# sandflow/ffmpeg-ht

Measured on AMD Instinct MI355X. Metric: Mpixels/s HTJ2K decode (4K lossless 5/3) at 1/2/4/8 GPU; IDWT HBM GB/s vs peak, higher is better.
Workload: dtype int32 (int16 storage); 1 GPU; configs[1]: 3840x2160 RGB 8-bit lossless 5/3 + RCT, 64x64 codeblocks, 5 levels, single tile, HT cleanup pass only; 128 frames per step per GPU as 2 concurrent jobs (HIP streams; the frame pipeline keeps that many in flight), device-resident input (codeblock bytes + descriptors) and output (rgb24); jobs=2, distinct_frames=4, block_errors=0

## Files before the change

ffmpeg-ht_amd/csrc/ht_kernels.hpp:

```cpp
#pragma once
#include <hip/hip_runtime.h>
#include <stdint.h>
#include "j2k_plan.h"

namespace htj2k {

struct HtLds {
    uint32_t off_ms, ms_words;
    uint32_t off_vlc, vlc_words;
    uint32_t off_suf, suf_bytes;
    uint32_t off_qinfo, max_qw;
    uint32_t off_E;
    uint32_t off_bm, bm_words;
    uint32_t total;
};

#define HT_ERR_INVALID 1
#define HT_REF_STRIDE 64
#define HT_MEL_SYMS  1344
#define HT_MEL_WORDS (HT_MEL_SYMS / 32 + 2)
#define HT_UVLC_ENTRIES (5 * 64)
#define HT_VSTAGE_PITCH 17
#define HT_VSTAGE_BYTES (64 * HT_VSTAGE_PITCH * 4)

typedef uint16_t ht_sym_t;
__host__ __device__ inline uint32_t ht_nsw(uint32_t Scup) { return (Scup * 8 + 31) / 32 + 2; }
__host__ __device__ inline uint32_t ht_nsp(uint32_t Lref) { return (Lref * 8 + 31) / 32 + 3; }

__host__ __device__ inline uint32_t ht_sym_pack_fields(uint32_t rho, uint32_t ek, uint32_t e1)
{
    uint32_t pk = 0;
    for (int n = 0; n < 4; n++) pk |= (((rho >> n) & 1) + ((ek >> n) & 1) + ((e1 >> n) & 1)) << (2 * n);
    return pk;
}
__device__ __forceinline__ uint32_t ht_sym_unpack(uint32_t s)
{
    const uint32_t pk = s & 0xFF, lo = pk & 0x55, hi = (pk >> 1) & 0x55;
    uint32_t t = (lo | hi) | (hi << 8) | ((lo & hi) << 16);
    t = (t | (t >> 1)) & 0x333333u;
    t = (t | (t >> 2)) & 0x0F0F0Fu;
    return (t & 0xF) | ((t >> 4) & 0xF0) | ((t >> 8) & 0xF00) | ((s >> 8) << 16);
}
__host__ __device__ inline uint32_t ht_qsym_pitch(uint32_t w) { return (((w + 1) >> 1) + 1) & ~1u; }
__host__ __device__ inline uint32_t ht_qsym_words(uint32_t w, uint32_t h) { return (ht_qsym_pitch(w) * ((h + 1) >> 1) + 15) & ~15u; }

__device__ __forceinline__ uint32_t wave_incl_scan_u32(uint32_t v, int lane)
{
    (void)lane;
    int x = (int)v;
    x += __builtin_amdgcn_update_dpp(0, x, 0x111, 0xf, 0xf, false);
    x += __builtin_amdgcn_update_dpp(0, x, 0x112, 0xf, 0xf, false);
    x += __builtin_amdgcn_update_dpp(0, x, 0x114, 0xf, 0xf, false);
    x += __builtin_amdgcn_update_dpp(0, x, 0x118, 0xf, 0xf, false);
    x += __builtin_amdgcn_update_dpp(0, x, 0x142, 0xa, 0xf, false);
    x += __builtin_amdgcn_update_dpp(0, x, 0x143, 0xc, 0xf, false);
    return (uint32_t)x;
}
__device__ __forceinline__ uint32_t wave_last(uint32_t v) { return (uint32_t)__builtin_amdgcn_readlane((int)v, 63); }

__device__ __forceinline__ void wave_lds_fence()
{
    __builtin_amdgcn_fence(__ATOMIC_ACQ_REL, "wavefront");
    __builtin_amdgcn_wave_barrier();
}

__device__ __forceinline__ void ht_ms_clear(uint32_t *p, uint32_t nwords, int lane)
{
    for (uint32_t i = 4u * lane; i < nwords; i += 256) *(uint4 *)(p + i) = make_uint4(0u, 0u, 0u, 0u);
}
__device__ __forceinline__ void ht_ms_ones_tail(uint32_t *p, uint32_t total, uint32_t last_word, int lane)
{
    for (uint32_t i = (total >> 5) + lane; i <= last_word; i += 64) {
        if (i * 32 >= total) p[i] = 0xFFFFFFFFu;
        else p[i] |= 0xFFFFFFFFu << (total & 31);
    }
}

__device__ __forceinline__ uint32_t ht_dequant(uint32_t smag, int transform, int M_b, int roi_shift,
                                               float fscale, int i_step)
{
    uint32_t mag = smag & 0x7FFFFFFFu;
    bool neg = (smag >> 31) != 0;
    if (roi_shift) {
        const uint32_t mask = 0xFFFFFFFFu >> (M_b + 1);
        if ((mag & ~mask) == 0) {
            const uint32_t v = mag << roi_shift;
            neg = neg || (v >> 31) != 0;
            mag = v & 0x7FFFFFFFu;
        }
    }
    if (transform == J2K_DWT53) {
        int v = (int)(mag >> (31 - M_b));
        if (neg) v = -v;
        if (i_step != 32768) {
            long long t = (long long)v * i_step;
            v = (int)(t < 0 ? -((-t) >> 16) : (t >> 16));
        }
        return (uint32_t)v;
    } else if (transform == J2K_DWT97) {
        int v = neg ? -(int)mag : (int)mag;
        return __float_as_uint((float)v * fscale);
    } else {
        int v = neg ? -(int)mag : (int)mag;
        v = (v + 32) >> 6;
        long long t = (long long)v * i_step;
        return (uint32_t)(int)((t + (1 << 15)) >> 16);
    }
}

struct HtSerial {
    uint64_t vbuf; int vbits; uint32_t vword;
    const uint32_t *vlc; uint32_t vlc_words;
    const uint8_t *suf; uint32_t mel_pos, mel_len; uint32_t mel_tmp; int mel_bits;
    int mel_k, mel_run, mel_one;

    __device__ __forceinline__ void vfill()
    {
        if (vbits <= 32) {
            uint32_t wv = vword < vlc_words ? vlc[vword] : 0u;
            vword++;
            vbuf |= (uint64_t)wv << vbits;
            vbits += 32;
        }
    }
    __device__ __forceinline__ uint32_t vpeek(int n) { vfill(); return (uint32_t)vbuf & ((1u << n) - 1); }
    __device__ __forceinline__ void vdrop(int n) { vbuf >>= n; vbits -= n; }
    __device__ __forceinline__ uint32_t vget(int n) { uint32_t v = vpeek(n); vdrop(n); return v; }

    __device__ __forceinline__ int mel_bit()
    {
        if (mel_bits == 0) {
            const bool cond = mel_pos < mel_len;
            mel_bits = (mel_tmp == 0xFF) ? 7 : 8;
            mel_tmp = cond ? suf[mel_pos] : 0xFFu;
            mel_pos += cond;
        }
        mel_bits--;
        return (mel_tmp >> mel_bits) & 1;
    }
    __device__ __forceinline__ int mel_sym()
    {
        static const uint8_t MEL_E[13] = { 0, 0, 0, 1, 1, 1, 2, 2, 2, 3, 3, 4, 5 };
        if (mel_run == 0 && mel_one == 0) {
            int eval = (0x5433222111000ull >> (4 * mel_k)) & 0xF;
            (void)MEL_E;
            if (mel_bit()) {
                mel_run = 1 << eval;
                mel_k = mel_k < 12 ? mel_k + 1 : 12;
            } else {
                mel_run = 0;
                while (eval > 0) { mel_run = 2 * mel_run + mel_bit(); eval--; }
                mel_run &= 0xFF;
                mel_k = mel_k > 0 ? mel_k - 1 : 0;
                mel_one = 1;
            }
        }
        if (mel_run > 0) { mel_run--; return 0; }
        mel_one = 0;
        return 1;
    }
    __device__ __forceinline__ int upfx()
    {
        uint32_t b = vpeek(3);
        int val  = (0x12131215u >> (4 * b)) & 0xF;
        int drop = (0x12131213u >> (4 * b)) & 0xF;
        vdrop(drop);
        return val;
    }
    __device__ __forceinline__ int usfx(int pfx)
    {
        if (pfx < 3) return 0;
        if (pfx == 3) return (int)vget(1);
        return (int)vget(5);
    }
    __device__ __forceinline__ int uext(int sfx) { return sfx >= 28 ? (int)vget(4) : 0; }
};

__device__ __forceinline__ void ht_zero_window(uint32_t *dst, int w, int h, int stride, int lane)
{
    for (int y = 0; y < h; y++)
// ... 1232 lines not shown
                }
                dst[(size_t)y * stride + x] = ht_dequant(v, transform, M_b, roi_shift, fscale, i_step);
            }
    }
}


__device__ __forceinline__ void ht_unstuff_backward_step8(uint2 dq, uint32_t k0, uint32_t n, uint32_t first_or,
                                                          uint32_t *out, int lane, uint32_t &base, uint32_t &carry)
{
    const uint32_t k = k0 + 8 * lane;
    uint32_t lo = __builtin_bswap32(dq.y), hi = __builtin_bswap32(dq.x);
    if (k == 0) lo |= first_or;
    int nv = 8;
    if (k0 + 512 > n) {
        nv = min(max((int)n - (int)k, 0), 8);
        const int nl = min(nv, 4), nh = nv - nl;
        lo = nl == 4 ? lo : (nl ? lo & (0xFFFFFFFFu >> (32 - 8 * nl)) : 0u);
        hi = nh == 4 ? hi : (nh ? hi & (0xFFFFFFFFu >> (32 - 8 * nh)) : 0u);
    }
    const uint32_t ll = lo & 0x7F7F7F7Fu, lh = hi & 0x7F7F7F7Fu;
    const uint32_t Al = (ll + 0x70707070u) & lo & 0x80808080u, Ah = (lh + 0x70707070u) & hi & 0x80808080u;
    const uint32_t Bl = (ll + 0x01010101u) & 0x80808080u, Bh = (lh + 0x01010101u) & 0x80808080u;
    uint32_t prevA = ht_dpp_left(Ah >> 24);
    if (lane == 0) prevA = carry;
    carry = (uint32_t)__builtin_amdgcn_readlane((int)(Ah >> 24), 63);
    uint32_t fl = Bl & ((Al << 8) | prevA), fh = Bh & __builtin_amdgcn_alignbyte(Ah, Al, 3);
    if (nv < 8) {
        const int nl = min(nv, 4), nh = nv - nl;
        fl = nl == 4 ? fl : (nl ? fl & (0xFFFFFFFFu >> (32 - 8 * nl)) : 0u);
        fh = nh == 4 ? fh : (nh ? fh & (0xFFFFFFFFu >> (32 - 8 * nh)) : 0u);
    }
    ht_squeeze_place<false>(lo, hi, fl, fh, nv, out, lane, base);
}

__device__ __forceinline__ uint32_t ht_unstuff_backward(const uint8_t *__restrict__ top, uint32_t n, uint32_t first_or,
                                                        uint32_t *out, int lane)
{
    uint32_t base = 0, carry = 0x80;
    for (uint32_t k0 = 0; k0 < n; k0 += 512) {
        const uint32_t k = k0 + 8 * lane;
        uint2 dq = make_uint2(0u, 0u);
        if (k < n) __builtin_memcpy(&dq, top - k - 7, 8);
        ht_unstuff_backward_step8(dq, k0, n, first_or, out, lane, base, carry);
    }
    return base;
}

__device__ __forceinline__ uint32_t ht_unstuff_forward7(const uint8_t *__restrict__ src, uint32_t n, uint32_t *out, int lane)
{
    uint32_t base = 0, carry = 0;
    for (uint32_t p0 = 0; p0 * 8 < n; p0 += 64) {
        const uint32_t i = (p0 + lane) * 8;
        uint2 dq = make_uint2(0u, 0u);
        if (i < n) __builtin_memcpy(&dq, src + i, 8);
        ht_unstuff_fwd_step8<false>(dq, p0, n, out, lane, base, carry);
    }
    return base;
}


template <int LPB>
__device__ __forceinline__ uint32_t grp_incl_scan_u32(uint32_t v)
{
    int x = (int)v;
    x += __builtin_amdgcn_update_dpp(0, x, 0x111, 0xf, 0xf, false);
    x += __builtin_amdgcn_update_dpp(0, x, 0x112, 0xf, 0xf, false);
    x += __builtin_amdgcn_update_dpp(0, x, 0x114, 0xf, 0xf, false);
    x += __builtin_amdgcn_update_dpp(0, x, 0x118, 0xf, 0xf, false);
    if (LPB >= 32) x += __builtin_amdgcn_update_dpp(0, x, 0x142, 0xa, 0xf, false);
    if (LPB >= 64) x += __builtin_amdgcn_update_dpp(0, x, 0x143, 0xc, 0xf, false);
    return (uint32_t)x;
}
template <int LPB>
__device__ __forceinline__ uint32_t grp_last(uint32_t v, int lane)
{
    return (uint32_t)__builtin_amdgcn_ds_bpermute((lane | (LPB - 1)) << 2, (int)v);
}
template <bool OR_SEM, int LPB>
__device__ __forceinline__ void ht_squeeze_place_g(uint32_t lo, uint32_t hi, uint32_t fl, uint32_t fh, int nv,
                                                   uint32_t *out, int lane, uint32_t &base)
{
    const uint32_t tot = 8u * (uint32_t)nv - (uint32_t)__builtin_popcount(fl) - (uint32_t)__builtin_popcount(fh);
    while (__ballot(fh != 0) != 0) {
        if (fh) {
            const uint32_t k = 31u - (uint32_t)__builtin_clz(fh), bit = 1u << k, m = bit - 1u;
            uint32_t nh = (hi & m) | ((hi >> 1) & ~m);
            if (OR_SEM) nh |= hi & bit;
            hi = nh;
            fh &= m;
        }
    }
    while (__ballot(fl != 0) != 0) {
        if (fl) {
            const uint32_t k = 31u - (uint32_t)__builtin_clz(fl), bit = 1u << k, m = bit - 1u;
            uint32_t nl = (lo & m) | (__builtin_amdgcn_alignbit(hi, lo, 1) & ~m);
            if (OR_SEM) nl |= lo & bit;
            lo = nl;
            hi >>= 1;
            fl &= m;
        }
    }
    const uint32_t incl = grp_incl_scan_u32<LPB>(tot);
    const uint32_t off = base + incl - tot;
    if (nv > 0) {
        const uint32_t sh = off & 31;
        const uint64_t t = (uint64_t)lo << sh, u = (uint64_t)hi << sh;
        uint32_t *o = out + (off >> 5);
        atomicOr(o, (uint32_t)t);
        atomicOr(o + 1, (uint32_t)(t >> 32) | (uint32_t)u);
        if (sh + tot + (OR_SEM ? 1u : 0u) > 64) atomicOr(o + 2, (uint32_t)(u >> 32));
    }
    base += grp_last<LPB>(incl, lane);
}
__device__ __forceinline__ uint32_t ht_first_bytes(uint32_t v, int n) { return n >= 4 ? v : (n > 0 ? v & (0xFFFFFFFFu >> (32 - 8 * n)) : 0u); }
template <int LPB>
__device__ __forceinline__ void ht_unstuff_backward_step8_g(uint2 dq, uint32_t k0, uint32_t n, uint32_t first_or,
                                                            uint32_t *out, int lane, uint32_t &base, uint32_t &carry)
{
    const int gl = lane & (LPB - 1);
    const uint32_t k = k0 + 8 * gl;
    const int nv = min(max((int)n - (int)k, 0), 8);
    uint32_t lo = __builtin_bswap32(dq.y), hi = __builtin_bswap32(dq.x);
    if (k == 0) lo |= first_or;
    lo = ht_first_bytes(lo, nv); hi = ht_first_bytes(hi, nv - 4);
    const uint32_t ll = lo & 0x7F7F7F7Fu, lh = hi & 0x7F7F7F7Fu;
    const uint32_t Al = (ll + 0x70707070u) & lo & 0x80808080u, Ah = (lh + 0x70707070u) & hi & 0x80808080u;
    const uint32_t Bl = (ll + 0x01010101u) & 0x80808080u, Bh = (lh + 0x01010101u) & 0x80808080u;
    uint32_t prevA = ht_dpp_left(Ah >> 24);
    if (gl == 0) prevA = carry;
    carry = grp_last<LPB>(Ah >> 24, lane);
    const uint32_t fl = ht_first_bytes(Bl & ((Al << 8) | prevA), nv), fh = ht_first_bytes(Bh & __builtin_amdgcn_alignbyte(Ah, Al, 3), nv - 4);
    ht_squeeze_place_g<false, LPB>(lo, hi, fl, fh, nv, out, lane, base);
}
template <int LPB>
__device__ __forceinline__ void ht_unstuff_fwd7_step8_g(uint2 dq, uint32_t p0, uint32_t n, uint32_t *out, int lane,
                                                        uint32_t &base, uint32_t &carry)
{
    const int gl = lane & (LPB - 1);
    const int nv = min(max((int)n - (int)(p0 + 8 * gl), 0), 8);
    const uint32_t lo = ht_first_bytes(dq.x, nv), hi = ht_first_bytes(dq.y, nv - 4);
    uint32_t prev = ht_dpp_left(hi >> 24);
    if (gl == 0) prev = carry;
    carry = grp_last<LPB>(hi >> 24, lane);
    const uint32_t Pl = (lo << 8) | prev, Ph = __builtin_amdgcn_alignbyte(hi, lo, 3);
    const uint32_t fl = ht_first_bytes(((Pl & 0x7F7F7F7Fu) + 0x01010101u) & Pl & 0x80808080u, nv);
    const uint32_t fh = ht_first_bytes(((Ph & 0x7F7F7F7Fu) + 0x01010101u) & Ph & 0x80808080u, nv - 4);
    ht_squeeze_place_g<false, LPB>(lo, hi, fl, fh, nv, out, lane, base);
}

template <int LPB>
__global__ void __launch_bounds__(64)
k_ht_unstuff_g(const J2kBlock *__restrict__ blocks, int nblocks, const uint8_t *__restrict__ bytes,
               uint32_t *__restrict__ vlc_u, uint32_t *__restrict__ mel_u, uint32_t lds_words)
{
    extern __shared__ __align__(16) uint32_t sw[];
    constexpr int G = 64 / LPB;
    const int lane = threadIdx.x, gl = lane & (LPB - 1);
    const int bi = (int)blockIdx.x * G + lane / LPB;
    J2kBlock b;
    memset(&b, 0, sizeof(b));
    if (bi < nblocks) b = blocks[bi];
    const uint8_t *D = bytes + b.data_off;
    const uint32_t Lcup = b.lcup;
    bool ok = bi < nblocks && b.npasses != 0 && Lcup >= 2;
    uint2 pv[2];
#pragma unroll
    for (int j = 0; j < 2; j++) {
        const long long o = (long long)b.data_off + Lcup - 9 - (8 * LPB * j + 8 * gl);
        pv[j] = make_uint2(0u, 0u);
        if (ok && o >= 0) __builtin_memcpy(&pv[j], bytes + o, 8);
    }
    uint32_t Scup = 0;
    if (ok) Scup = ((uint32_t)D[Lcup - 1] << 4) + (D[Lcup - 2] & 0x0F);
    ok = ok && !(Scup < 2 || Scup > Lcup || Scup > 4079);
    const uint32_t nsw = ht_nsw(Scup);
    ok = ok && 2 * nsw <= lds_words;
    uint32_t *vlO = vlc_u + (b.data_off >> 2), *meO = mel_u + (b.data_off >> 2);
    uint32_t *sv = sw + (size_t)(lane / LPB) * lds_words;

    if (ok) for (uint32_t i = gl; i < nsw; i += LPB) sv[i] = 0;
    __syncthreads();
    {
        const uint8_t *top = D + Lcup - 2;
        const uint32_t n = ok ? Scup - 1 : 0u;
        uint32_t base = 0, carry = 0x80;
#pragma unroll
        for (int j = 0; j < 2; j++)
            if (__ballot((uint32_t)(8 * LPB * j) < n) != 0) ht_unstuff_backward_step8_g<LPB>(pv[j], 8 * LPB * j, n, 0x0F, sv, lane, base, carry);
        for (uint32_t k0 = 16 * LPB; __ballot(k0 < n) != 0; k0 += 8 * LPB) {
            const uint32_t k = k0 + 8 * gl;
            uint2 dq = make_uint2(0u, 0u);
            if (k < n) __builtin_memcpy(&dq, top - k - 7, 8);
            ht_unstuff_backward_step8_g<LPB>(dq, k0, n, 0x0F, sv, lane, base, carry);
        }
    }
    __syncthreads();
    if (ok) for (uint32_t i = gl; i < nsw; i += LPB) vlO[i] = sv[i];

    const int rem = b.npasses % 3, plhd = rem ? b.npasses - rem : b.npasses - 3;
    const uint32_t Lref = b.lref, nsp = ht_nsp(Lref);
    const bool ref = ok && b.npasses - plhd > 1 && Lref > 0 && 2 * nsp <= lds_words;
    if (__ballot(ref) == 0) return;
    uint32_t *ss = sv, *sr = sv + nsp;
    __syncthreads();
    if (ref) for (uint32_t i = gl; i < 2 * nsp; i += LPB) sv[i] = 0;
    __syncthreads();
    {
        const uint32_t n = ref ? Lref : 0u;
        uint32_t base = 0, carry = 0;
        for (uint32_t p0 = 0; __ballot(p0 < n) != 0; p0 += 8 * LPB) {
            const uint32_t i = p0 + 8 * gl;
            uint2 dq = make_uint2(0u, 0u);
            if (i < n) __builtin_memcpy(&dq, D + Lcup + i, 8);
            ht_unstuff_fwd7_step8_g<LPB>(dq, p0, n, ss, lane, base, carry);
        }
        base = 0; carry = 0x80;
        const uint8_t *top = D + Lcup + Lref - 1;
        for (uint32_t k0 = 0; __ballot(k0 < n) != 0; k0 += 8 * LPB) {
            const uint32_t k = k0 + 8 * gl;
            uint2 dq = make_uint2(0u, 0u);
            if (k < n) __builtin_memcpy(&dq, top - k - 7, 8);
            ht_unstuff_backward_step8_g<LPB>(dq, k0, n, 0, sr, lane, base, carry);
        }
    }
    __syncthreads();
    if (ref) for (uint32_t i = gl; i < nsp; i += LPB) {
        vlO[nsw + i] = ss[i];
        meO[nsw + i] = sr[i];
    }
}

__global__ void __launch_bounds__(64)
k_ht_unstuff(const J2kBlock *__restrict__ blocks, int nblocks, const uint8_t *__restrict__ bytes,
             uint32_t *__restrict__ vlc_u, uint32_t *__restrict__ mel_u, uint32_t lds_words)
{
    extern __shared__ __align__(16) uint32_t sw[];
    const int lane = threadIdx.x;
    if ((int)blockIdx.x >= nblocks) return;
    const J2kBlock b = blocks[blockIdx.x];
    if (b.npasses == 0 || b.lcup < 2) return;
    const uint8_t *D = bytes + b.data_off;
    const uint32_t Lcup = b.lcup;
    uint2 pv[2];
#pragma unroll
    for (int j = 0; j < 2; j++) {
        const long long o = (long long)b.data_off + Lcup - 9 - (512 * j + 8 * lane);
        pv[j] = make_uint2(0u, 0u);
        if (o >= 0) __builtin_memcpy(&pv[j], bytes + o, 8);
    }
    const uint32_t Scup = (uint32_t)__builtin_amdgcn_readfirstlane((int)(((uint32_t)D[Lcup - 1] << 4) + (D[Lcup - 2] & 0x0F)));
    if (Scup < 2 || Scup > Lcup || Scup > 4079) return;
    const uint32_t nsw = ht_nsw(Scup);
    if (2 * nsw > lds_words) return;
    uint32_t *vlO = vlc_u + (b.data_off >> 2), *meO = mel_u + (b.data_off >> 2);
    uint32_t *sv = sw;

    for (uint32_t i = lane; i < nsw; i += 64) sw[i] = 0;
    __syncthreads();

    {
        const uint8_t *top = D + Lcup - 2;
        const uint32_t n = Scup - 1;
        uint32_t base = 0, carry = 0x80;
#pragma unroll
        for (int j = 0; j < 2; j++)
            if (512u * j < n) ht_unstuff_backward_step8(pv[j], 512 * j, n, 0x0F, sv, lane, base, carry);
        for (uint32_t k0 = 1024; k0 < n; k0 += 512) {
            const uint32_t k = k0 + 8 * lane;
            uint2 dq = make_uint2(0u, 0u);
            if (k < n) __builtin_memcpy(&dq, top - k - 7, 8);
            ht_unstuff_backward_step8(dq, k0, n, 0x0F, sv, lane, base, carry);
        }
    }

    __syncthreads();
    for (uint32_t i = lane; i < nsw; i += 64) vlO[i] = sv[i];

    const int rem = b.npasses % 3, plhd = rem ? b.npasses - rem : b.npasses - 3;
    if (b.npasses - plhd > 1 && b.lref > 0) {
        const uint32_t Lref = b.lref, nsp = ht_nsp(Lref);
        if (2 * nsp > lds_words) return;
        uint32_t *ss = sw, *sr = sw + nsp;
        __syncthreads();
        for (uint32_t i = lane; i < 2 * nsp; i += 64) sw[i] = 0;
        __syncthreads();
        ht_unstuff_forward7(D + Lcup, Lref, ss, lane);
        ht_unstuff_backward(D + Lcup + Lref - 1, Lref, 0, sr, lane);
        __syncthreads();
        for (uint32_t i = lane; i < nsp; i += 64) {
            vlO[nsw + i] = ss[i];
            meO[nsw + i] = sr[i];
        }
    }
}

template <typename MT, bool MAGREF>
__global__ void __launch_bounds__(64, (sizeof(MT) == 4 && !MAGREF) ? 6 : 4)
k_ht_refine(const J2kBlock *__restrict__ blocks, const uint32_t *__restrict__ ref_list, int nref,
            const uint8_t *__restrict__ bytes, const ht_sym_t *__restrict__ qsym, const uint32_t *__restrict__ qoff,
            const uint32_t *__restrict__ vlc_u, const uint32_t *__restrict__ mel_u,
            uint64_t *__restrict__ refbits, const uint32_t *__restrict__ roff)
{
    constexpr int MB = (int)sizeof(MT) * 8;
    const int li = blockIdx.x * 64 + threadIdx.x;
    if (li >= nref) return;
    const uint32_t bi = ref_list[li];
    const J2kBlock b = blocks[bi];
    const int w = b.w, h = b.h, qw = (w + 1) >> 1, qh = (h + 1) >> 1;
    uint64_t *out = refbits + roff[bi];
    for (int y = 0; y < 3 * h; y++) out[(size_t)y * HT_REF_STRIDE] = 0;
    if (b.npasses == 0 || b.lcup < 2 || w > MB) return;
    const uint8_t *D = bytes + b.data_off;
    const uint32_t Scup = ((uint32_t)D[b.lcup - 1] << 4) + (D[b.lcup - 2] & 0x0F);
    if (Scup < 2 || Scup > b.lcup || Scup > 4079) return;
    const int rem = b.npasses % 3, plhd = rem ? b.npasses - rem : b.npasses - 3;
    const int z_blk = b.npasses - plhd;
    if (z_blk <= 1) return;
    const bool causal = (b.flags & J2K_CBLK_VSC) != 0;
    const ht_sym_t *qs = qsym + qoff[bi];
    const uint32_t nsw = ht_nsw(Scup), nsp = b.lref ? ht_nsp(b.lref) : 0;
    const uint32_t *spw = vlc_u + (b.data_off >> 2) + nsw, *mrw = mel_u + (b.data_off >> 2) + nsw;
    const MT wmask = w >= MB ? (MT)~(MT)0 : (MT)(((MT)1 << w) - 1);

    struct Bits {
        const uint32_t *p; uint32_t n, idx; uint64_t buf; int cnt; uint32_t q0, q1, q2, q3, left; uint4 nx;
        __device__ __forceinline__ uint4 fetch(uint32_t i) const
        {
            uint4 v = make_uint4(0u, 0u, 0u, 0u);
            if (i < n) {
                __builtin_memcpy(&v, p + i, 16);
                if (i + 1 >= n) v.y = 0;
                if (i + 2 >= n) v.z = 0;
                if (i + 3 >= n) v.w = 0;
            }
            return v;
        }
        __device__ __forceinline__ void init(const uint32_t *q, uint32_t nw)
        {
            p = q; n = nw; buf = 0; cnt = 0;
            const uint4 v = fetch(0);
            q0 = v.x; q1 = v.y; q2 = v.z; q3 = v.w; left = 4;
            nx = fetch(4); idx = 8;
        }
        __device__ __forceinline__ void top_up()
        {
            buf |= (uint64_t)q0 << cnt;
            cnt += 32;
            q0 = q1; q1 = q2; q2 = q3;
            if (--left == 0) {
                q0 = nx.x; q1 = nx.y; q2 = nx.z; q3 = nx.w; left = 4;
                nx = fetch(idx); idx += 4;
            }
        }
        __device__ __forceinline__ uint32_t get()
        {
            const uint32_t bit = (uint32_t)buf & 1u;
            buf >>= 1; cnt--;
            return bit;
        }
    } sp, mr;
    sp.init(spw, nsp);
    if (MAGREF) mr.init(mrw, nsp);

    const uint32_t qpitch = ht_qsym_pitch((uint32_t)w);
    auto two_quads = [](uint32_t s2, int q, MT &top, MT &bot) {
        const uint32_t r2 = (s2 | (s2 >> 1)) & 0x00550055u;
        top |= (MT)((r2 & 1u) | ((r2 >> 3) & 2u) | ((r2 >> 14) & 4u) | ((r2 >> 17) & 8u)) << (2 * q);
        bot |= (MT)(((r2 >> 2) & 1u) | ((r2 >> 5) & 2u) | ((r2 >> 16) & 4u) | ((r2 >> 19) & 8u)) << (2 * q);
    };
    auto quad_rows = [&](int qy, MT &top, MT &bot) {
        top = 0; bot = 0;
        if (qy >= qh) return;
        const uint32_t *row = (const uint32_t *)(qs + (size_t)qy * qpitch);
        if ((qpitch & 7) == 0) {
            for (int q = 0; q < qw; q += 8) {
                const uint4 s8 = *(const uint4 *)(row + (q >> 1));
                two_quads(s8.x, q, top, bot);
                two_quads(s8.y, q + 2, top, bot);
                two_quads(s8.z, q + 4, top, bot);
                two_quads(s8.w, q + 6, top, bot);
            }
        } else {
            for (int q = 0; q < qw; q += 2) two_quads(row[q >> 1], q, top, bot);
        }
        top &= wmask; bot &= wmask;
        if (2 * qy + 1 >= h) bot = 0;
    };

    MT a_top, a_bot;
    quad_rows(0, a_top, a_bot);
    MT Mup = 0;
    for (int i0 = 0; i0 < h; i0 += 4) {
        MT b_top, b_bot, c_top, c_bot;
        quad_rows(i0 / 2 + 1, b_top, b_bot);
        quad_rows(i0 / 2 + 2, c_top, c_bot);
        const MT S0 = a_top, S1 = a_bot, S2 = b_top, S3 = b_bot, S4 = c_top;
        MT R0 = 0, R1 = 0, R2 = 0, R3 = 0, G0 = 0, G1 = 0, G2 = 0, G3 = 0, Q0 = 0, Q1 = 0, Q2 = 0, Q3 = 0;
        const int gh = min(4, h - i0);
        {
            auto smear = [](MT x) -> MT { return x | (MT)(x << 1) | (x >> 1); };
            const bool dn0 = !causal || gh != 1, dn1 = !causal || gh != 2, dn2 = !causal || gh != 3, dn3 = !causal || gh != 4;
            MT s0 = S0, s1 = S1, s2 = S2, s3 = S3;
            MT T0 = smear(Mup) | (MT)(S0 << 1) | (S0 >> 1) | (dn0 ? smear(S1) : (MT)0);
            MT T1 = smear(S0) | (MT)(S1 << 1) | (S1 >> 1) | (dn1 ? smear(S2) : (MT)0);
            MT T2 = smear(S1) | (MT)(S2 << 1) | (S2 >> 1) | (dn2 ? smear(S3) : (MT)0);
            MT T3 = smear(S2) | (MT)(S3 << 1) | (S3 >> 1) | (dn3 ? smear(S4) : (MT)0);
            const uint32_t m0 = dn0 ? 7u : 3u, m1 = dn1 ? 7u : 3u, m2 = dn2 ? 7u : 3u, m3 = dn3 ? 7u : 3u;
            uint32_t rprev = 0;
            for (int j0 = 0; j0 < w; j0 += 4) {
                uint32_t rc4[4] = { 0, 0, 0, 0 };
                if (sp.cnt <= 32) sp.top_up();
#pragma unroll
                for (int jj = 0; jj < 4; jj++) {
                    const int j = j0 + jj;
                    if (j < w) {
                        const uint32_t RP = rprev << 1;
                        uint32_t rcur = 0;
                        if (gh > 0 && !((uint32_t)s0 & 1u) && ((((uint32_t)T0 & 1u) | (RP & m0)) != 0) && sp.get()) rcur |= 1u;
                        if (gh > 1 && !((uint32_t)s1 & 1u) && ((((uint32_t)T1 & 1u) | ((RP >> 1) & m1) | (rcur & 1u)) != 0) && sp.get()) rcur |= 2u;
                        if (gh > 2 && !((uint32_t)s2 & 1u) && ((((uint32_t)T2 & 1u) | ((RP >> 2) & m2) | (rcur & 2u)) != 0) && sp.get()) rcur |= 4u;
                        if (gh > 3 && !((uint32_t)s3 & 1u) && ((((uint32_t)T3 & 1u) | ((RP >> 3) & m3) | (rcur & 4u)) != 0) && sp.get()) rcur |= 8u;
                        R0 |= (MT)(rcur & 1u) << j; R1 |= (MT)((rcur >> 1) & 1u) << j;
                        R2 |= (MT)((rcur >> 2) & 1u) << j; R3 |= (MT)(rcur >> 3) << j;
                        rc4[jj] = rcur;
                        rprev = rcur;
                        s0 >>= 1; s1 >>= 1; s2 >>= 1; s3 >>= 1;
                        T0 >>= 1; T1 >>= 1; T2 >>= 1; T3 >>= 1;
                    }
                }
// ... 175 lines not shown
            uint64_t mw;
            uint32_t n7 = 0;
            if (!slow) {
                const uint32_t hi = __builtin_amdgcn_perm(pfB, pfA, 0x01020304u), lo = __builtin_amdgcn_perm(pfC, pfB, 0x01020304u);
                mw = (((uint64_t)hi << 32) | lo) << o;
            } else {
                uint32_t prev = 0, total = 0;
                mw = 0;
#pragma unroll
                for (int j = -1; j < 7; j++) {
                    const int p = mb + j;
                    const uint32_t raw = ((j < 3 ? pfA >> (8 * (j + 1)) : pfB >> (8 * (j - 3)))) & 0xFF;
                    const uint32_t v = p >= mlim - 1 ? 0xFFu : (p == mlim - 2 ? raw | 0x0Fu : raw);
                    if (j >= 0) {
                        const uint32_t n = prev == 0xFF ? 7u : 8u;
                        mw = (mw << n) | (v & ((1u << n) - 1));
                        total += n;
                        n7 |= (8u - n) << j;
                    }
                    prev = p < 0 ? 0u : v;
                }
                mw <<= (64 - total) + (o - (n7 & 1));
            }
            uint32_t used_all = 0;
#pragma unroll
            for (int cw = 0; cw < 6; cw++) {
                const int eval = (int)((0x5433222111000ull >> (4 * mel_k)) & 0xF);
                const int b = (int)(mw >> 63);
                const int run = b ? (1 << eval) : (eval ? (int)((mw << 1) >> (64 - eval)) : 0);
                const int nsy = run + (b ? 0 : 1);
                if (mcnt + nsy <= 64) {
                    if (!b) msyms |= 1ull << ((mcnt + run) & 63);
                    mcnt += nsy;
                    const int used = b ? 1 : 1 + eval;
                    mw <<= used; used_all += used;
                    mel_k = b ? (mel_k < 12 ? mel_k + 1 : 12) : (mel_k > 0 ? mel_k - 1 : 0);
                }
            }
            if (!slow) {
                mrb += used_all;
            } else {
                uint32_t L = 0, before = 0, cum = 8 - o;
#pragma unroll
                for (int j = 0; j < 6; j++) {
                    const bool ge = used_all >= cum;
                    L += ge;
                    before = ge ? cum : before;
                    cum += 8 - ((n7 >> (j + 1)) & 1);
                }
                mrb = L ? (uint32_t)(mb + (int)L) * 8 + ((n7 >> L) & 1) + (used_all - before) : mrb + used_all;
            }
            const uint8_t *pm = mraw + min((int)(mrb >> 3), mlim) - 1;
            __builtin_memcpy(&pfA, pm, 4);
            __builtin_memcpy(&pfB, pm + 4, 4);
            __builtin_memcpy(&pfC, pm + 8, 4);
        }
        uint64_t vwin;
        {
            const uint32_t kw = (vpos >> 5) & 15, sh = vpos & 31;
            const uint32_t a0 = vst[kw], a1 = vst[(kw + 1) & 15], a2 = vst[(kw + 2) & 15];
            vwin = ((uint64_t)__builtin_amdgcn_alignbit(a2, a1, sh) << 32) | __builtin_amdgcn_alignbit(a1, a0, sh);
        }
        uint32_t m = (uint32_t)msyms, mused = 0;
        uint32_t a = (uint32_t)vwin, aused = 0;
        int rho[2], uoff[2];
        uint32_t pk[2];
#pragma unroll
        for (int k = 0; k < 2; k++) {
            const bool en = active && (k == 0 || pair);
            const int q = qx + k;
            const int ra = ra_next;
            const int rar = (row && en && q + 1 < qw) ? (int)myrho[q + 1] : 0;
            const int ctx = row0 ? ctx_run
                                 : ((((ra >> 1) | (ral >> 3)) & 1) | ((((rho_left >> 2) | (rho_left >> 3)) & 1) << 1) |
                                    ((((ra >> 3) | (rar >> 1)) & 1) << 2));
            const bool mq = en && ctx == 0;
            const int msym = (int)(m & 1);
            m >>= mq ? 1 : 0; mused += mq ? 1 : 0;
            const bool dec = en && (ctx != 0 || msym != 0);
            const uint32_t e = dec ? table[(ctx << 7) | (a & 0x7F)] : 0u;
            const uint32_t len = (e >> 1) & 7;
            a >>= len; aused += len;
            uoff[k] = e & 1; rho[k] = (e >> 4) & 0xF; pk[k] = e >> 8;
            if (en) {
                rho_left = rho[k];
                ral = ra;
                ra_next = rar;
                ctx_run = ((rho[k] | (rho[k] >> 1)) & 1) | (((rho[k] >> 2) & 1) << 1) | (((rho[k] >> 3) & 1) << 2);
            }
        }
        uint32_t u32w = (uint32_t)(vwin >> aused), uused;
        const bool both = uoff[0] && uoff[1];
        const bool mq2 = row0 && both;
        const int mel2 = (int)(m & 1);
        mused += mq2 ? 1 : 0;
        const int mode = (mq2 && !mel2) ? 4 : (uoff[0] | (uoff[1] << 1));
        const uint32_t ue = utbl[(mode << 6) | (u32w & 63)];
        const int p1 = ue & 7, p2 = (ue >> 3) & 7;
        uint32_t d = (ue >> 6) & 7;
        u32w >>= d; uused = d;
        d = (ue >> 9) & 7;
        const int s1 = (int)(u32w & ((1u << d) - 1)); u32w >>= d; uused += d;
        d = (ue >> 12) & 7;
        const int s2 = (int)(u32w & ((1u << d) - 1)); u32w >>= d; uused += d;
        d = s1 >= 28 ? 4u : 0u;
        const int x1 = (int)(u32w & ((1u << d) - 1)); u32w >>= d; uused += d;
        d = s2 >= 28 ? 4u : 0u;
        const int x2 = (int)(u32w & ((1u << d) - 1)); uused += d;
        const int bias = (mq2 && mel2) ? 2 : 0;
        const int u1 = uoff[0] ? bias + p1 + s1 + 4 * x1 : 0;
        const int u2 = uoff[1] ? bias + p2 + s2 + 4 * x2 : 0;
        if (active) {
            vpos += aused + uused;
            msyms >>= mused; mcnt -= (int)mused;
            myrho[qx] = (uint8_t)rho[0];
            if (pair) myrho[qx + 1] = (uint8_t)rho[1];
        }
        ost[t & (CAD - 1)] = pk[0] | ((uint32_t)u1 << 8) | (pk[1] << 16) | ((uint32_t)u2 << 24);
        qx += 2;
        if (active && qx >= qw) {
            qx = 0; row++;
            rho_left = 0; ral = 0;
            ra_next = (int)myrho[0];
        }
    }
    if (max_it > 0) flush((max_it - 1) / CAD);
}


#define HT_VLC2_VPITCH 18
#define HT_VLC2_LDS (4096 + 1024 + HT_VLC_NARROW_WAVES * 64 * (HT_VLC2_VPITCH + HT_VLC_OUT_PITCH) * 4)

__host__ __device__ inline uint32_t ht_uvlc_entry2_from(uint32_t p1, uint32_t p2, uint32_t lp, uint32_t d1, uint32_t d2)
{
    return lp | (d1 << 5) | (p1 << 8) | ((lp + d1) << 11) | (d2 << 16) | ((lp + d1 + d2) << 19) | (p2 << 24);
}
__host__ __device__ inline uint32_t ht_uvlc_entry2(int mode, uint32_t v)
{
    const uint32_t e = ht_uvlc_entry(mode, v);
    return ht_uvlc_entry2_from(e & 7, (e >> 3) & 7, (e >> 6) & 7, (e >> 9) & 7, (e >> 12) & 7);
}
__device__ __forceinline__ uint32_t ht_uvlc_entry2_mode4(uint32_t v)
{
    const uint32_t b = v & 7;
    const uint32_t p1 = (0x12131215u >> (4 * b)) & 0xF;
    uint32_t lp = (0x12131213u >> (4 * b)) & 0xF, p2;
    if (p1 > 2) { p2 = ((v >> lp) & 1) + 1; lp += 1; }
    else { const uint32_t b2 = (v >> lp) & 7; p2 = (0x12131215u >> (4 * b2)) & 0xF; lp += (0x12131213u >> (4 * b2)) & 0xF; }
    const uint32_t d1 = p1 < 3 ? 0u : (p1 == 3 ? 1u : 5u);
    const uint32_t d2 = p1 > 2 ? 0u : (p2 < 3 ? 0u : (p2 == 3 ? 1u : 5u));
    return ht_uvlc_entry2_from(p1, p2, lp, d1, d2);
}

__global__ void __launch_bounds__(64 * HT_VLC_NARROW_WAVES)
k_ht_vlc2(const J2kBlock *__restrict__ blocks, int nblocks, const uint8_t *__restrict__ bytes,
          const uint16_t *__restrict__ g_tables, ht_sym_t *__restrict__ qsym,
          const uint32_t *__restrict__ qoff,
          const uint32_t *__restrict__ vlc_u, uint32_t *__restrict__ sink)
{
    extern __shared__ __align__(16) uint8_t smem[];
    uint16_t *tbl = (uint16_t *)smem;
    uint32_t *utbl = (uint32_t *)(smem + 4096);
    constexpr int CAD = 8;
    constexpr int VPITCH = HT_VLC2_VPITCH, OPITCH = HT_VLC_OUT_PITCH;
    const int lane = threadIdx.x & 63, wv = threadIdx.x >> 6;
    uint32_t *vstage = (uint32_t *)(smem + 4096 + 1024) + wv * 64 * (VPITCH + OPITCH);
    uint32_t *ostage = vstage + 64 * VPITCH;
    const int bi = blockIdx.x * blockDim.x + threadIdx.x;
    for (int i = threadIdx.x; i < 2048; i += blockDim.x) {
        const uint32_t e = g_tables[i], rho = (e >> 4) & 0xF;
        const uint32_t ne = (e & 0xF) | (((rho >> 1) & 1) << 4) | (((rho >> 3) & 1) << 5) | ((((rho >> 2) | (rho >> 3)) & 1) << 6) |
                            (ht_sym_pack_fields(rho, (e >> 8) & 0xF, (e >> 12) & 0xF) << 8);
        const int ctx = (i >> 7) & 7, bits = i & 127;
        const int dst = i < 1024 ? i : 1024 + (bits | ((ctx & 1) << 7) | (((ctx >> 2) & 1) << 8) | (((ctx >> 1) & 1) << 9));
        tbl[dst] = (uint16_t)ne;
    }
    for (int i = threadIdx.x; i < 4 * 64; i += blockDim.x)
        utbl[i] = ht_uvlc_entry2(i >> 6, (uint32_t)(i & 63));

    int qw = 0, qh = 0;
    uint32_t doff = 0;
    ht_sym_t *qout = qsym;
    const uint8_t *mraw = bytes + 16;
    int mlim = 0;
    if (bi < nblocks) {
        const J2kBlock b = blocks[bi];
        bool ok = b.npasses != 0 && b.lcup >= 2;
        uint32_t Scup = 0;
        if (ok) {
            const uint8_t *D = bytes + b.data_off;
            Scup = ((uint32_t)D[b.lcup - 1] << 4) + (D[b.lcup - 2] & 0x0F);
            ok = !(Scup < 2 || Scup > b.lcup || Scup > 4079);
        }
        if (ok && ((b.w + 1u) >> 1) <= 32u) {
            qw = (b.w + 1) >> 1;
            qh = (b.h + 1) >> 1;
            qout = qsym + qoff[bi];
            doff = b.data_off >> 2;
            mraw = bytes + b.data_off + (b.lcup - Scup);
            mlim = (int)Scup;
        }
    }
    const int ppr = (qw + 1) >> 1;
    const int n_it = qh * ppr;
    int max_it = n_it;
#pragma unroll
    for (int o = 32; o; o >>= 1) max_it = max(max_it, __shfl_xor(max_it, o));
    const uint32_t my_lo = (uint32_t)(uintptr_t)qout, my_hi = (uint32_t)((uintptr_t)qout >> 32);
    __syncthreads();

    const uint32_t *vsrc = vlc_u + doff;
    uint32_t vpos = 4;
    uint32_t *vst = vstage + lane * VPITCH;
    uint32_t *ost = ostage + lane * OPITCH;
    uint4 nxv = make_uint4(0u, 0u, 0u, 0u), nxw = make_uint4(0u, 0u, 0u, 0u);
    uint32_t hw = 16, pw = 0;
    bool pend = false;
    uint64_t msyms = 0; int mcnt = 0; uint32_t mrb = 0; int mel_k = 0;
    uint32_t pfA, pfB, pfC;
    __builtin_memcpy(&pfA, mraw - 1, 4);
    __builtin_memcpy(&pfB, mraw + 3, 4);
    __builtin_memcpy(&pfC, mraw + 7, 4);
    if (qh > 0) {
#pragma unroll
        for (int jx = 0; jx < 4; jx++) {
            uint4 q;
            __builtin_memcpy(&q, vsrc + 4 * jx, 16);
            vst[4 * jx] = q.x; vst[4 * jx + 1] = q.y; vst[4 * jx + 2] = q.z; vst[4 * jx + 3] = q.w;
            if (jx == 0) { vst[16] = q.x; vst[17] = q.y; }
        }
    }
    auto flush = [&](int win) {
#pragma unroll
        for (int p = 0; p < 2; p++) {
            const int c = 32 * p + (lane >> 1), part = lane & 1;
            const uint32_t *src = ostage + c * OPITCH + 4 * part;
            const uint4 v = make_uint4(src[0], src[1], src[2], src[3]);
            const uint32_t c_lo = (uint32_t)__builtin_amdgcn_ds_bpermute(4 * c, (int)my_lo);
            const uint32_t c_hi = (uint32_t)__builtin_amdgcn_ds_bpermute(4 * c, (int)my_hi);
            const uint32_t c_nit = (uint32_t)__builtin_amdgcn_ds_bpermute(4 * c, n_it);
            uint32_t *dst = (uint32_t *)(((uintptr_t)c_hi << 32) | c_lo) + (size_t)win * CAD + 4 * part;
            typedef uint32_t u32x4 __attribute__((ext_vector_type(4)));
            typedef __attribute__((address_space(1))) u32x4 g_u32x4;
            u32x4 vv; vv.x = v.x; vv.y = v.y; vv.z = v.z; vv.w = v.w;
            *(g_u32x4 *)(uintptr_t)((uint32_t)(win * CAD) < c_nit ? dst : sink + 4 * part) = vv;
        }
    };

    int row = 0, qx = 0;
    uint32_t ctx_run = 0;
    uint32_t lf10 = 0;
    uint32_t Dlo = 0, Dhi = 0, Mlo = 0, Mhi = 0;
    const uint8_t *tb1 = (const uint8_t *)(tbl + 1024);
    auto pass = [&](int t, auto main_tag) {
        constexpr bool MAIN = decltype(main_tag)::value;
        const bool active = MAIN || t < n_it;
        const bool row0 = !MAIN && row == 0;
        const bool pair = MAIN || qx + 1 < qw;
        if ((t & 1) == 0) {
            if (pend) {
                uint32_t *r = vst + (pw & 15);
                r[0] = nxv.x; r[1] = nxv.y; r[2] = nxv.z; r[3] = nxv.w;
                if (!(pw & 15)) { vst[16] = nxv.x; vst[17] = nxv.y; }
                r = vst + ((pw + 4) & 15);
                r[0] = nxw.x; r[1] = nxw.y; r[2] = nxw.z; r[3] = nxw.w;
            }
            pend = (int)(hw - (vpos >> 5)) < 8;
            if (pend) {
                __builtin_memcpy(&nxv, vsrc + hw, 16);
                __builtin_memcpy(&nxw, vsrc + hw + 4, 16);
                pw = hw;
                hw += 8;
            }
            if ((t & (CAD - 1)) == 0 && t) flush(t / CAD - 1);
        }
        if (__ballot(mcnt < 3) != 0 && mcnt <= 32) {
            const int mb = (int)(mrb >> 3);
            const uint32_t o = mrb & 7;
            const uint32_t a0 = mb ? pfA : (pfA & ~0xFFu);
            const uint32_t anyff = ((~a0 - 0x01010101u) & a0 & 0x80808080u) | ((~pfB - 0x01010101u) & pfB & 0x80808080u);
            const bool slow = anyff != 0 || mb + 10 > mlim;
            uint64_t mw;
            uint32_t n7 = 0;
            if (!slow) {
                const uint32_t hi = __builtin_amdgcn_perm(pfB, pfA, 0x01020304u), lo = __builtin_amdgcn_perm(pfC, pfB, 0x01020304u);
                mw = (((uint64_t)hi << 32) | lo) << o;
            } else {
                uint32_t prev = 0, total = 0;
                mw = 0;
#pragma unroll
                for (int j = -1; j < 7; j++) {
                    const int p = mb + j;
                    const uint32_t raw = ((j < 3 ? pfA >> (8 * (j + 1)) : pfB >> (8 * (j - 3)))) & 0xFF;
                    const uint32_t v = p >= mlim - 1 ? 0xFFu : (p == mlim - 2 ? raw | 0x0Fu : raw);
                    if (j >= 0) {
                        const uint32_t n = prev == 0xFF ? 7u : 8u;
                        mw = (mw << n) | (v & ((1u << n) - 1));
                        total += n;
                        n7 |= (8u - n) << j;
                    }
                    prev = p < 0 ? 0u : v;
                }
                mw <<= (64 - total) + (o - (n7 & 1));
            }
            uint32_t used_all = 0;
#pragma unroll
            for (int cw = 0; cw < 6; cw++) {
                const int eval = (int)((0x5433222111000ull >> (4 * mel_k)) & 0xF);
                const int b = (int)(mw >> 63);
                const int run = b ? (1 << eval) : (eval ? (int)((mw << 1) >> (64 - eval)) : 0);
                const int nsy = run + (b ? 0 : 1);
                if (mcnt + nsy <= 64) {
                    if (!b) msyms |= 1ull << ((mcnt + run) & 63);
                    mcnt += nsy;
                    const int used = b ? 1 : 1 + eval;
                    mw <<= used; used_all += used;
                    mel_k = b ? (mel_k < 12 ? mel_k + 1 : 12) : (mel_k > 0 ? mel_k - 1 : 0);
                }
            }
            if (!slow) {
                mrb += used_all;
            } else {
                uint32_t L = 0, before = 0, cum = 8 - o;
#pragma unroll
                for (int j = 0; j < 6; j++) {
                    const bool ge = used_all >= cum;
                    L += ge;
                    before = ge ? cum : before;
                    cum += 8 - ((n7 >> (j + 1)) & 1);
                }
                mrb = L ? (uint32_t)(mb + (int)L) * 8 + ((n7 >> L) & 1) + (used_all - before) : mrb + used_all;
            }
            const uint8_t *pm = mraw + min((int)(mrb >> 3), mlim) - 1;
            __builtin_memcpy(&pfA, pm, 4);
            __builtin_memcpy(&pfB, pm + 4, 4);
            __builtin_memcpy(&pfC, pm + 8, 4);
        }
        uint32_t lo, hi;
        {
            const uint32_t *wp = (const uint32_t *)((const uint8_t *)vst + ((vpos >> 3) & 60u));
            const uint32_t a0 = wp[0], a1 = wp[1], a2 = wp[2];
            lo = __builtin_amdgcn_alignbit(a1, a0, vpos);
            hi = __builtin_amdgcn_alignbit(a2, a1, vpos);
        }
        uint32_t m = (uint32_t)msyms;
        uint32_t e0, e1, mused;
        {
            const bool en0 = active;
            uint32_t ad = row0 ? ((lo & 0x7Fu) << 1) | (ctx_run << 8)
                               : ((lo & 0x7Fu) << 1) | ((Dlo & 3u) << 8) | lf10;
            const uint32_t mq = (en0 && ad < 0x100u) ? 1u : 0u;
            const uint32_t et = *(const uint16_t *)((row0 ? (const uint8_t *)tbl : tb1) + ad);
            e0 = __umul24(et, (m | ~mq) & (MAIN ? 1u : (uint32_t)en0));
            m >>= mq; mused = mq;
            if (row0) {
                const uint32_t f = e0 >> 8, tt = (f | (f >> 1)) & 0x55u;
                if (en0) ctx_run = ((tt | (tt >> 2)) & 1u) | ((tt >> 3) & 2u) | ((tt >> 4) & 4u);
            }
            const bool en1 = active && pair;
            const uint32_t len0 = (e0 >> 1) & 7u;
            const uint32_t bits1 = __builtin_amdgcn_ubfe(lo, len0, 7u) << 1;
            ad = row0 ? bits1 | (ctx_run << 8) : bits1 | ((Dlo & 0xCu) << 6) | ((e0 & 0x40u) << 4);
            const uint32_t mq1 = (en1 && ad < 0x100u) ? 1u : 0u;
            const uint32_t et1 = *(const uint16_t *)((row0 ? (const uint8_t *)tbl : tb1) + ad);
            e1 = __umul24(et1, (m | ~mq1) & (MAIN ? 1u : (uint32_t)en1));
            m >>= mq1; mused += mq1;
            if (row0) {
                const uint32_t f = e1 >> 8, tt = (f | (f >> 1)) & 0x55u;
                if (en1) ctx_run = ((tt | (tt >> 2)) & 1u) | ((tt >> 3) & 2u) | ((tt >> 4) & 4u);
            }
            if (MAIN || en1) lf10 = (e1 & 0x40u) << 4;
            else if (en0) lf10 = (e0 & 0x40u) << 4;
            const uint32_t X = ((e0 >> 4) & 3u) | (((e1 >> 4) & 3u) << 2);
            const uint32_t sh = MAIN ? 4u : 2u * ((uint32_t)en0 + (uint32_t)en1);
            Mlo = __builtin_amdgcn_alignbit(Mhi, Mlo, sh);
            Mhi = __builtin_amdgcn_alignbit(X, Mhi, sh);
            Dlo = __builtin_amdgcn_alignbit(Dhi, Dlo, 4u);
            Dhi >>= 4;
        }
        const uint32_t aused = ((e0 >> 1) & 7u) + ((e1 >> 1) & 7u);
        const uint32_t w = __builtin_amdgcn_alignbit(hi, lo, aused);
        uint32_t ue = utbl[(w & 63u) | ((e0 & 1u) << 6) | ((e1 & 1u) << 7)];
        uint32_t bias = 0;
        if (!MAIN) {
            const bool mq2 = row0 && (e0 & e1 & 1u);
            if (__ballot(mq2) != 0) {
                const uint32_t mel2 = m & 1u;
                if (mq2) {
                    mused += 1;
                    if (mel2) bias = 0x02000200u; else ue = ht_uvlc_entry2_mode4(w & 63u);
                }
            }
        }
        const uint32_t s1 = __builtin_amdgcn_ubfe(w, ue, __builtin_amdgcn_ubfe(ue, 5u, 3u));
        const uint32_t s2 = __builtin_amdgcn_ubfe(w, ue >> 11, __builtin_amdgcn_ubfe(ue, 16u, 3u));
        uint32_t uused = __builtin_amdgcn_ubfe(ue, 19u, 5u);
        uint32_t out = __builtin_amdgcn_perm(e1, e0, 0x0C050C01u) + (ue & 0x07000700u) + (s1 << 8) + (s2 << 24) + bias;
        if (__ballot(s1 >= 28u || s2 >= 28u) != 0) {
            const uint32_t d1x = s1 >= 28u ? 4u : 0u, d2x = s2 >= 28u ? 4u : 0u;
            const uint32_t x1 = __builtin_amdgcn_ubfe(w, uused, d1x), x2 = __builtin_amdgcn_ubfe(w, uused + d1x, d2x);
            out += (x1 << 10) + (x2 << 26);
            uused += d1x + d2x;
        }
        if (active) {
            vpos += aused + uused;
            msyms >>= mused; mcnt -= (int)mused;
        }
        ost[t & (CAD - 1)] = out;
        qx += 2;
        if (active && qx >= qw) {
            const uint64_t I = (((uint64_t)Mhi << 32) | Mlo) >> (64 - 2 * qw);
            const uint64_t Dn = ((I | (I << 1)) & 0x5555555555555555ull) | ((I | (I >> 1)) & 0xAAAAAAAAAAAAAAAAull);
            Dlo = (uint32_t)Dn; Dhi = (uint32_t)(Dn >> 32);
            Mlo = 0; Mhi = 0;
            qx = 0; row++;
            lf10 = 0; ctx_run = 0;
        }
    };
    int t_a = ppr, t_b = n_it, odd = qw & 1;
#pragma unroll
    for (int o = 32; o; o >>= 1) {
        t_a = max(t_a, __shfl_xor(t_a, o));
        t_b = min(t_b, __shfl_xor(t_b, o));
// ... 12 lines not shown
```

ffmpeg-ht_amd/csrc/htj2k_device.hip:

```cpp
#include <hip/hip_runtime.h>
#include <stdarg.h>
#include <stdio.h>
#include <stdlib.h>
#include <string.h>
#include <algorithm>
#include <atomic>
#include <chrono>
#include <mutex>
#include <thread>
#include <vector>

#include "../../include/htj2k_amd.h"
#include "j2k_plan.h"
#include "ht_cxtvlc_rows.h"
#include "ht_kernels.hpp"
#include "dwt_kernels.hpp"
#include "pack_kernels.hpp"
#include "dwt_stream.hpp"
#include "mq_kernels.hpp"

using namespace htj2k;

__global__ void __launch_bounds__(256) k_gather(const J2kSeg *__restrict__ segs, const uint32_t *__restrict__ first_seg, int ngroups,
                                                 const uint8_t *__restrict__ pkt, const uint8_t *__restrict__ lit,
                                                 uint8_t *__restrict__ pool)
{
    const int g = blockIdx.x * 4 + (threadIdx.x >> 6), lane = threadIdx.x & 63;
    if (g >= ngroups) return;
    const uint32_t s1 = first_seg[g + 1];
    for (uint32_t s = first_seg[g]; s < s1; s++) {
        const J2kSeg sg = segs[s];
        const uint8_t *src = ((sg.flags & J2K_SEG_LIT) ? lit : pkt) + sg.src;
        uint8_t *dst = pool + sg.dst;
        const uint32_t head = min(sg.len, (uint32_t)(-(intptr_t)dst & 3));
        if ((uint32_t)lane < head) dst[lane] = src[lane];
        const uint32_t body = (sg.len - head) >> 2, tail0 = head + 4 * body;
        const uint8_t *bs = src + head;
        const uint32_t sh = (uint32_t)((uintptr_t)bs & 3);
        const uint32_t *al = (const uint32_t *)(bs - sh);
        uint32_t *out = (uint32_t *)(dst + head);
        for (uint32_t k = lane; k < body; k += 64) {
            const uint32_t lo = al[k], hi = sh ? al[k + 1] : 0u;
            out[k] = __builtin_amdgcn_alignbyte(hi, lo, sh);
        }
        if ((uint32_t)lane < sg.len - tail0) dst[tail0 + lane] = src[tail0 + lane];
        if ((sg.flags & J2K_SEG_TERM) && lane < 2) dst[sg.len + lane] = 0xFF;
    }
}

#define LOG_ERROR 16
#define LOG_WARNING 24
#define LOG_INFO 32

struct DevBuf {
    void *p = nullptr;
    size_t cap = 0;
    int ensure(size_t n)
    {
        if (n <= cap) return 0;
        if (p) (void)hipFree(p);
        p = nullptr; cap = 0;
        size_t want = n + n / 8 + 256;
        if (hipMalloc(&p, want) != hipSuccess) { p = nullptr; return HTJ2K_ERR_ENOMEM; }
        cap = want;
        static const bool poison = getenv("HTJ2K_POISON") && atoi(getenv("HTJ2K_POISON"));
        if (poison) {
            (void)hipMemset(p, 0xA5, want);
            (void)hipDeviceSynchronize();
        }
        return 0;
    }
    void release() { if (p) (void)hipFree(p); p = nullptr; cap = 0; }
};

struct HostBuf {
    void *p = nullptr;
    size_t cap = 0;
    int device = 0;
    void *ensure(size_t n)
    {
        if (n <= cap) return p;
        if (hipSetDevice(device) != hipSuccess) return nullptr;
        if (p) (void)hipHostFree(p);
        p = nullptr; cap = 0;
        const size_t want = n + n / 4 + 4096;
        if (hipHostMalloc(&p, want, hipHostMallocDefault) != hipSuccess) { p = nullptr; return nullptr; }
        cap = want;
        return p;
    }
    void release() { if (p) (void)hipHostFree(p); p = nullptr; cap = 0; }
};

struct htj2k_ctx {
    htj2k_opts opts;
    int device = 0;
    char devname[256];
    htj2k_log_fn log = nullptr;
    void *log_opaque = nullptr;
    uint16_t *d_tables = nullptr;
    J2kParser *probe_parser = nullptr;
    htj2k_job *own_job = nullptr;
    int idwt_mode = 3;
    int fuse_pack = 1;
    int idwt_x3 = 1;
    int ht_pair = 1;
    int ht_multi = 1;
    int idwt_pk = 1;
    int ll16_test_bits = 16;
    int ll16 = 1;
    int coef16 = 1;
    int ht_mode = 1;
    int max_dyn_lds = 64 * 1024;
    int parse_threads = 0;
    int packet_threads = 1;
    int device_gather = 1;
    std::mutex log_mutex;
    std::atomic<int> refs{1};
};

struct LevelLaunch {
    int type, level;
    int count;
    size_t table_off;
    int max_lh, max_lv, min_l;
    double alg_bytes;
    double hbm_bytes = 0;
    int nc = 0;
    int outk = -1;
    bool all_fast = false;
    int pk_bits = 0;
};

struct FrameSlot {
    J2kParser *parser = nullptr;
    const J2kPlan *plan = nullptr;
    HostBuf h_pkt;
    const uint8_t *h2d_src = nullptr;
    bool h2d_own = false;
    size_t pkt_base = 0;
    HostBuf h_bytes;
    float ms_stage = 0, ms_parse = 0;
    uint32_t block_base = 0, tc_base = 0, sample_base = 0;
    size_t bytes_base = 0;
    DevBuf d_out[4];
    OutPlanes out;
};

struct htj2k_job {
    std::vector<FrameSlot> frames;
    int nframes = 0;
    std::vector<J2kBlock> blocks;
    std::vector<J2kTileComp> tilecomps;
    std::vector<int> tc_frame;
    size_t nbytes = 0, nsamples = 0;
    hipStream_t stream = nullptr;
    hipEvent_t ev[6] = { nullptr, nullptr, nullptr, nullptr, nullptr, nullptr };
    std::vector<hipEvent_t> lev_ev;
    int lev_ev_used = 0;
    std::vector<double> lev_bytes, lev_hbm;
    DevBuf d_bytes, d_blocks, d_status, d_coef, d_t0, d_t1, d_desc, d_qsym, d_qoff, d_vlcu, d_melu, d_reflist, d_roff, d_refbits;
    bool pair_ok = false;
    int multi_nb = 0;
    int multi_t = 0;
    bool coef16_ok = false;
    bool coef_is16 = false;
    int ht_bpw = 0;
    bool ll16_run = false;
    bool ll16_checked = true;
    bool force_ll32 = false;
    int ll16_fallbacks = 0;
    int nht = 0;
    std::vector<MqWave> mqwaves;
    size_t mq_scratch_units = 0;
    uint32_t mq_planes = 1;
    DevBuf d_mqwaves, d_mqscratch;
    bool dev_gather = false;
    DevBuf d_pkt, d_lit, d_gsegs, d_ggroups;
    std::vector<J2kSeg> gsegs;
    std::vector<uint32_t> ggroups;
    std::vector<uint8_t> lit;
    size_t pkt_bytes = 0;
    bool pkt_h2d_issued = false;
    std::vector<uint32_t> qoff;
    std::vector<uint32_t> reflist, roff;
    size_t nrefmasks = 0;
    uint32_t ref_max_w = 0;
    uint32_t ref_max_h = 0;
    uint32_t max_lref = 0;
    size_t nquads = 0;
    HtLds lds_ext;
    uint32_t max_qw = 1;
    std::vector<uint8_t> h_desc;
    std::vector<uint8_t> h_desc_dev;
    std::vector<LevelLaunch> launches_generic, launches_tile;
    std::vector<LevelLaunch> launches_fused;
    std::vector<uint8_t> tile_fusable;
    std::vector<uint8_t> plane_fused;
    bool any_fusable = false;
    int pk_used = 0;
    bool pk_run = false;
    int pk_bits = 0;
    bool x3_ok = false;
    size_t x3_tab[3] = { 0, 0, 0 };
    int x3_count = 0, x3_lh[3] = { 0, 0, 0 }, x3_lv2 = 0;
    double x3_alg = 0, x3_hbm = 0;
    bool fused_last = false;
    size_t pack_off = 0; int npack = 0; int pack_maxw = 0, pack_maxh = 0;
    HtLds lds;
    int uploaded = 0, ran = 0;
    std::vector<int> final_buf;
    std::vector<int> final_eff;
    bool tile_ok = true;
};

static void clog(htj2k_ctx *c, int level, const char *fmt, ...)
{
    char buf[512];
    va_list ap;
    if (!c || !c->log) return;
    va_start(ap, fmt);
    vsnprintf(buf, sizeof buf, fmt, ap);
    va_end(ap);
    c->log(c->log_opaque, level, buf);
}

static void parser_log_tramp(void *opaque, int level, const char *msg)
{
    htj2k_ctx *c = (htj2k_ctx *)opaque;
    if (c && c->log) {
        std::lock_guard<std::mutex> lk(c->log_mutex);
        c->log(c->log_opaque, level, msg);
    }
}

#define HIP_TRY(c, expr)                                                                      \
    do {                                                                                      \
        hipError_t e_ = (expr);                                                               \
        if (e_ != hipSuccess) {                                                               \
            clog(c, LOG_ERROR, "HIP error %s at %s:%d (%s)\n", hipGetErrorString(e_), __FILE__, __LINE__, #expr); \
            return e_ == hipErrorOutOfMemory ? HTJ2K_ERR_ENOMEM : HTJ2K_ERR_EXTERNAL;         \
        }                                                                                     \
    } while (0)

static uint16_t h_tables[2][1024];
static void tbl_row(int t, int ctx, int rho, int uoff, int ek, int e1, int cwd, int len)
{
    uint16_t v = (uint16_t)(uoff | (len << 1) | (rho << 4) | (ek << 8) | (e1 << 12));
    for (int hi = 0; hi < (1 << (7 - len)); hi++)
        h_tables[t][(ctx << 7) | (hi << len) | cwd] = v;
}
#define DROW0(c, r, u, k, o, w, l) tbl_row(0, c, r, u, k, o, w, l);
#define DROW1(c, r, u, k, o, w, l) tbl_row(1, c, r, u, k, o, w, l);
static void build_tables()
{
    HT_CXTVLC_ROWS0(DROW0)
    HT_CXTVLC_ROWS1(DROW1)
}

extern "C" const char *htj2k_version(void) { return "htj2k-amd 0.1 (gfx950)"; }

extern "C" int htj2k_open(const htj2k_opts *opts, htj2k_ctx **out)
{
    int ndev = 0;
    if (!out) return HTJ2K_ERR_EINVAL;
    *out = nullptr;
    if (hipGetDeviceCount(&ndev) != hipSuccess || ndev <= 0)
        return HTJ2K_ERR_ENOSYS;
    htj2k_ctx *c = new (std::nothrow) htj2k_ctx();
    if (!c) return HTJ2K_ERR_ENOMEM;
    memset(&c->opts, 0, sizeof(c->opts));
    c->opts.req_pix_fmt = HTJ2K_PIX_NONE;
    if (opts) c->opts = *opts;
    c->device = c->opts.device_id;
    if (c->device < 0 || c->device >= ndev) { delete c; return HTJ2K_ERR_EINVAL; }
    if (hipSetDevice(c->device) != hipSuccess) { delete c; return HTJ2K_ERR_ENOSYS; }
    hipDeviceProp_t prop;
    if (hipGetDeviceProperties(&prop, c->device) != hipSuccess) { delete c; return HTJ2K_ERR_ENOSYS; }
    snprintf(c->devname, sizeof(c->devname), "%s", prop.gcnArchName);
    c->max_dyn_lds = (int)prop.sharedMemPerBlock;
    build_tables();
    if (hipMalloc((void **)&c->d_tables, sizeof(h_tables)) != hipSuccess ||
        hipMemcpy(c->d_tables, h_tables, sizeof(h_tables), hipMemcpyHostToDevice) != hipSuccess) {
        delete c;
        return HTJ2K_ERR_ENOSYS;
    }
    c->probe_parser = j2k_parser_new();
    if (!c->probe_parser) { (void)hipFree(c->d_tables); delete c; return HTJ2K_ERR_ENOMEM; }
    const char *hm = getenv("HTJ2K_HT");
    if (hm && !strcmp(hm, "fused")) c->ht_mode = 0;
    if (hm && !strcmp(hm, "split")) c->ht_mode = 1;
    const char *m = getenv("HTJ2K_IDWT");
    if (m && !strcmp(m, "generic")) c->idwt_mode = 0;
    if (m && !strcmp(m, "tile")) c->idwt_mode = 1;
    if (m && !strcmp(m, "stream")) c->idwt_mode = 3;
    const char *l16 = getenv("HTJ2K_LL16");
    if (l16) c->ll16 = atoi(l16) ? 1 : 0;
    const char *pk = getenv("HTJ2K_PK");
    if (pk) c->idwt_pk = atoi(pk) ? 1 : 0;
    const char *fz = getenv("HTJ2K_FUSE");
    if (fz) c->fuse_pack = atoi(fz) != 0;
    *out = c;
    return 0;
}

extern "C" void htj2k_set_log(htj2k_ctx *c, htj2k_log_fn fn, void *opaque)
{
    if (!c) return;
    c->log = fn;
    c->log_opaque = opaque;
    j2k_parser_set_log(c->probe_parser, fn ? parser_log_tramp : nullptr, c);
}

extern "C" int htj2k_set_int(htj2k_ctx *c, const char *name, int value)
{
    if (!c || !name) return HTJ2K_ERR_EINVAL;
    if (!strcmp(name, "idwt_mode")) { c->idwt_mode = value <= 0 ? 0 : (value >= 3 ? 3 : 1); return 0; }
    if (!strcmp(name, "fuse_pack")) { c->fuse_pack = value ? 1 : 0; return 0; }
    if (!strcmp(name, "parse_threads")) { c->parse_threads = value < 0 ? 0 : (value > 64 ? 64 : value); return 0; }
    if (!strcmp(name, "ht_mode")) { c->ht_mode = value ? 1 : 0; return 0; }
    if (!strcmp(name, "device_gather")) { c->device_gather = value ? 1 : 0; return 0; }
    if (!strcmp(name, "packet_threads")) { c->packet_threads = value < 1 ? 1 : (value > 16 ? 16 : value); return 0; }
    if (!strcmp(name, "coef16")) { c->coef16 = value ? 1 : 0; return 0; }
    if (!strcmp(name, "ht_pair")) { c->ht_pair = value ? 1 : 0; return 0; }
    if (!strcmp(name, "idwt_x3")) { c->idwt_x3 = value ? 1 : 0; return 0; }
    if (!strcmp(name, "idwt_pk")) { c->idwt_pk = value ? 1 : 0; return 0; }
    if (!strcmp(name, "ht_multi")) { c->ht_multi = value ? 1 : 0; return 0; }
    if (!strcmp(name, "ll16")) { c->ll16 = value ? 1 : 0; return 0; }
    if (!strcmp(name, "ll16_test_bits")) { if (value < 2 || value > 16) return HTJ2K_ERR_EINVAL; c->ll16_test_bits = value; return 0; }
    if (!strcmp(name, "bitexact")) { c->opts.bitexact = value; return 0; }
    if (!strcmp(name, "reduction_factor")) { c->opts.reduction_factor = value; return 0; }
    return HTJ2K_ERR_EINVAL;
}

extern "C" const char *htj2k_device_name(htj2k_ctx *c) { return c ? c->devname : ""; }

extern "C" void *htj2k_host_alloc(htj2k_ctx *c, size_t size)
{
    void *p = nullptr;
    if (!c || !size || hipSetDevice(c->device) != hipSuccess) return nullptr;
    if (hipHostMalloc(&p, size, hipHostMallocDefault) != hipSuccess) return nullptr;
    return p;
}

extern "C" void htj2k_host_free(htj2k_ctx *c, void *ptr)
{
    (void)c;
    if (ptr) (void)hipHostFree(ptr);
}

extern "C" int htj2k_device_to_host(htj2k_ctx *c, void *dst, const void *src, size_t size)
{
    if (!c || !dst || !src) return HTJ2K_ERR_EINVAL;
    HIP_TRY(c, hipSetDevice(c->device));
    HIP_TRY(c, hipMemcpy(dst, src, size, hipMemcpyDeviceToHost));
    return 0;
}

extern "C" void htj2k_job_free(htj2k_ctx *c, htj2k_job *j)
{
    (void)c;
    if (!j) return;
    if (j->stream) (void)hipStreamSynchronize(j->stream);
    j->d_bytes.release(); j->d_blocks.release(); j->d_status.release(); j->d_coef.release();
    j->d_t0.release(); j->d_t1.release(); j->d_desc.release(); j->d_qsym.release(); j->d_qoff.release();
    j->d_vlcu.release(); j->d_melu.release(); j->d_reflist.release(); j->d_roff.release(); j->d_refbits.release();
    j->d_mqwaves.release(); j->d_mqscratch.release();
    j->d_pkt.release(); j->d_lit.release(); j->d_gsegs.release(); j->d_ggroups.release();
    for (FrameSlot &f : j->frames) {
        for (int i = 0; i < 4; i++) f.d_out[i].release();
        j2k_parser_free(f.parser);
        f.h_bytes.release();
        f.h_pkt.release();
    }
    for (int i = 0; i < 6; i++) if (j->ev[i]) (void)hipEventDestroy(j->ev[i]);
    for (hipEvent_t e : j->lev_ev) if (e) (void)hipEventDestroy(e);
    if (j->stream) (void)hipStreamDestroy(j->stream);
    delete j;
}

extern "C" void htj2k_ctx_ref_(htj2k_ctx *c) { if (c) c->refs.fetch_add(1); }
extern "C" int htj2k_ctx_default_depth_(const htj2k_ctx *c)
{
    const int d = c ? c->opts.frames_in_flight : 0;
    return d <= 0 ? 3 : (d > 16 ? 16 : d);
}

extern "C" void htj2k_close(htj2k_ctx *c)
{
    if (c && c->refs.fetch_sub(1) != 1) return;
    if (!c) return;
    (void)hipSetDevice(c->device);
    if (c->own_job) htj2k_job_free(c, c->own_job);
    if (c->d_tables) (void)hipFree(c->d_tables);
    j2k_parser_free(c->probe_parser);
    delete c;
}

extern "C" int htj2k_probe(htj2k_ctx *c, const uint8_t *pkt, int size, htj2k_info *info)
{
    const J2kPlan *pl = nullptr;
    if (!c || !pkt || !info) return HTJ2K_ERR_EINVAL;
    int ret = j2k_parse(c->probe_parser, pkt, size, &c->opts, 1, &pl);
    if (ret < 0) return ret;
    *info = pl->info;
    return 0;
}

static int job_new(htj2k_ctx *c, htj2k_job **out)
{
    htj2k_job *j = new (std::nothrow) htj2k_job();
    if (!j) return HTJ2K_ERR_ENOMEM;
    if (hipSetDevice(c->device) != hipSuccess || hipStreamCreateWithFlags(&j->stream, hipStreamNonBlocking) != hipSuccess) {
        delete j; return HTJ2K_ERR_EXTERNAL;
    }
    for (int i = 0; i < 6; i++)
        if (hipEventCreate(&j->ev[i]) != hipSuccess) { htj2k_job_free(c, j); return HTJ2K_ERR_EXTERNAL; }
    *out = j;
    return 0;
}

static hipError_t job_packet_h2d(htj2k_job *j, const FrameSlot &F, size_t size)
{
    uint8_t *dst = (uint8_t *)j->d_pkt.p + F.pkt_base;
    hipError_t e = hipMemcpyAsync(dst, F.h2d_src, size + (F.h2d_own ? 64 : 0), hipMemcpyHostToDevice, j->stream);
    if (e == hipSuccess && !F.h2d_own) e = hipMemsetAsync(dst + size, 0, 64, j->stream);
    return e;
}

extern "C" int htj2k_job_parse_batch(htj2k_ctx *c, const uint8_t *const *pkts, const int *sizes, int n, htj2k_job **job)
{
    return htj2k_job_parse_batch_ex(c, pkts, sizes, n, nullptr, job);
}

extern "C" int htj2k_job_parse_batch_ex(htj2k_ctx *c, const uint8_t *const *pkts, const int *sizes, int n, const uint8_t *pinned,
                                        htj2k_job **job)
{
    if (!c || !pkts || !sizes || n <= 0 || !job) return HTJ2K_ERR_EINVAL;
    if (!*job) {
        int r = job_new(c, job);
        if (r < 0) return r;
    }
    htj2k_job *j = *job;
    if (hipStreamSynchronize(j->stream) != hipSuccess) return HTJ2K_ERR_EXTERNAL;
    j->uploaded = j->ran = 0;
    j->nframes = 0;
    if ((int)j->frames.size() < n) j->frames.resize(n);
    j->blocks.clear(); j->tilecomps.clear(); j->tc_frame.clear();
    size_t nbytes = 0, nsamples = 0;
    j->dev_gather = c->device_gather != 0;
    for (int f = 0; f < n; f++) {
        FrameSlot &F = j->frames[f];
        if (!F.parser) {
            F.parser = j2k_parser_new();
            if (!F.parser) return HTJ2K_ERR_ENOMEM;
            j2k_parser_set_log(F.parser, parser_log_tramp, c);
        }
        F.h_bytes.device = c->device;
        F.h_pkt.device = c->device;
        j2k_parser_set_gather(F.parser, !j->dev_gather);
        j2k_parser_set_packet_threads(F.parser, n == 1 ? c->packet_threads : 1);
        j2k_parser_set_bytes_alloc(F.parser, [](void *opaque, size_t nb) -> void * { return ((HostBuf *)opaque)->ensure(nb); },
                                   &F.h_bytes);
        F.plan = nullptr;
    }
    {
        std::vector<int> rc(n, 0);
        int nthreads = c->parse_threads > 0 ? c->parse_threads : (int)std::min(16u, std::max(1u, std::thread::hardware_concurrency()));
        if (nthreads > n) nthreads = n;
        auto parallel_frames = [&](auto &&fn) {
            std::atomic<int> next(0);
            auto work = [&]() {
                for (;;) {
                    const int f = next.fetch_add(1);
                    if (f >= n) break;
                    fn(f);
                }
            };
            if (nthreads <= 1) {
                work();
            } else {
                std::vector<std::thread> pool;
                for (int t = 1; t < nthreads; t++) pool.emplace_back(work);
                work();
                for (std::thread &t : pool) t.join();
            }
        };
        const bool stage = j->dev_gather;
        std::vector<const uint8_t *> src(pkts, pkts + n);
        bool solo_done = false;
        if (stage && n == 1 && !(pinned && pinned[0]) && sizes[0] >= (4 << 20) && hipSetDevice(c->device) == hipSuccess) {
            FrameSlot &F = j->frames[0];
            const size_t sz = (size_t)sizes[0];
            const auto t0 = std::chrono::steady_clock::now();
            uint8_t *h = (uint8_t *)F.h_pkt.ensure(sz + 64);
            if (!h) return HTJ2K_ERR_ENOMEM;
            if (j->d_pkt.ensure(((sz + 64 + 15) & ~(size_t)15) + 256) == 0) {
                F.pkt_base = 0;
                F.h2d_src = h; F.h2d_own = true;
                const size_t piece = 2 << 20, npieces = (sz + piece - 1) / piece;
                const int nhelp = (int)std::min<size_t>(3, std::max(1u, std::thread::hardware_concurrency()) > 1 ? 3 : 1);
                std::atomic<size_t> nextp(0);
                std::atomic<int> bad(0);
                auto copy_pieces = [&]() {
                    if (hipSetDevice(c->device) != hipSuccess) { bad = 1; return; }
                    for (;;) {
                        const size_t k = nextp.fetch_add(1);
                        if (k >= npieces) break;
                        const size_t off = k * piece, len = std::min(piece, sz - off), pad = k + 1 == npieces ? 64 : 0;
                        memcpy(h + off, pkts[0] + off, len);
                        if (pad) memset(h + sz, 0, 64);
                        if (hipMemcpyAsync((uint8_t *)j->d_pkt.p + off, h + off, len + pad, hipMemcpyHostToDevice, j->stream) != hipSuccess) bad = 1;
                    }
                };
                std::vector<std::thread> helpers;
                for (int t = 0; t < nhelp; t++) helpers.emplace_back(copy_pieces);
                const auto t1 = std::chrono::steady_clock::now();
                rc[0] = j2k_parse(F.parser, pkts[0], sizes[0], &c->opts, 0, &F.plan);
                F.ms_parse = std::chrono::duration<float, std::milli>(std::chrono::steady_clock::now() - t1).count();
// ... 3 lines not shown
                if (rc[0] < 0) return rc[0];
                j->pkt_h2d_issued = true;
                solo_done = true;
            }
        }
        if (solo_done) {
        } else {
        if (stage)
            parallel_frames([&](int f) {
                FrameSlot &F = j->frames[f];
                const auto t0 = std::chrono::steady_clock::now();
                F.h2d_src = nullptr;
                F.h2d_own = false;
                if (pinned && pinned[f]) {
                    F.h2d_src = src[f];
                } else {
                    const size_t sz = sizes[f] > 0 ? (size_t)sizes[f] : 0;
                    uint8_t *h = (uint8_t *)F.h_pkt.ensure(sz + 64);
                    if (!h) { rc[f] = HTJ2K_ERR_ENOMEM; return; }
                    memcpy(h, src[f], sz);
                    memset(h + sz, 0, 64);
                    src[f] = h;
                    F.h2d_src = h;
                    F.h2d_own = true;
                }
                F.ms_stage = std::chrono::duration<float, std::milli>(std::chrono::steady_clock::now() - t0).count();
            });
        for (int f = 0; f < n; f++)
            if (rc[f] < 0) return rc[f];
        j->pkt_h2d_issued = false;
        if (stage) {
            size_t total = 0;
            bool fits = true;
            for (int f = 0; f < n; f++) {
                j->frames[f].pkt_base = total;
                total += ((size_t)(sizes[f] > 0 ? sizes[f] : 0) + 64 + 15) & ~(size_t)15;
                if (total > 0xFFFFFF00ull) fits = false;
            }
            if (fits && hipSetDevice(c->device) == hipSuccess && j->d_pkt.ensure(total + 256) == 0) {
                bool ok = true;
                for (int f = 0; f < n && ok; f++) ok = job_packet_h2d(j, j->frames[f], sizes[f] > 0 ? (size_t)sizes[f] : 0) == hipSuccess;
                j->pkt_h2d_issued = ok;
            }
        }
        parallel_frames([&](int f) {
            FrameSlot &F = j->frames[f];
            const auto t1 = std::chrono::steady_clock::now();
            rc[f] = j2k_parse(F.parser, src[f], sizes[f], &c->opts, 0, &F.plan);
            F.ms_parse = std::chrono::duration<float, std::milli>(std::chrono::steady_clock::now() - t1).count();
            if (!stage) F.ms_stage = 0;
        });
        for (int f = 0; f < n; f++)
            if (rc[f] < 0) return rc[f];
        }
    }
    j->gsegs.clear(); j->ggroups.clear(); j->lit.clear();
    size_t pkt_bytes = 0;
    for (int f = 0; f < n; f++) {
        FrameSlot &F = j->frames[f];
        const J2kPlan *pl = F.plan;
        if (nsamples + pl->nsamples > 0xFFFFFF00ull || nbytes + pl->nbytes > 0xFFFFFF00ull)
            return HTJ2K_ERR_PATCHWELCOME;
        F.block_base = (uint32_t)j->blocks.size();
        F.tc_base = (uint32_t)j->tilecomps.size();
        F.sample_base = (uint32_t)nsamples;
        nbytes += 16;
        F.bytes_base = nbytes;
        for (int i = 0; i < pl->nblocks; i++) {
            J2kBlock b = pl->blocks[i];
            b.data_off += (uint32_t)nbytes;
            b.plane_off += (uint32_t)nsamples;
            b.tcomp = (uint8_t)(b.tcomp + F.tc_base);
            j->blocks.push_back(b);
        }
        for (int t = 0; t < pl->ntilecomps; t++) {
            J2kTileComp tc = pl->tilecomps[t];
            tc.plane_off += (uint32_t)nsamples;
            j->tilecomps.push_back(tc);
            j->tc_frame.push_back(f);
        }
        if (j->dev_gather) {
            if (pkt_bytes + (size_t)pl->pkt_size > 0xFFFFFF00ull || j->lit.size() + pl->nlit > 0xFFFFFF00ull ||
                j->gsegs.size() + pl->nsegs > 0xFFFFFF00ull)
                return HTJ2K_ERR_PATCHWELCOME;
            if (F.pkt_base != pkt_bytes) j->pkt_h2d_issued = false;
            F.pkt_base = pkt_bytes;
            const uint32_t lit_base = (uint32_t)j->lit.size(), seg_base = (uint32_t)j->gsegs.size();
            for (uint32_t k = 0; k < pl->nsegs; k++) {
                J2kSeg g = pl->segs[k];
                g.src += (g.flags & J2K_SEG_LIT) ? lit_base : (uint32_t)pkt_bytes;
                g.dst += (uint32_t)nbytes;
                j->gsegs.push_back(g);
            }
            for (int i = 0; i < pl->nblocks; i++) j->ggroups.push_back(seg_base + pl->blk_seg0[i]);
            j->lit.insert(j->lit.end(), pl->lit, pl->lit + pl->nlit);
            pkt_bytes += ((size_t)pl->pkt_size + 64 + 15) & ~(size_t)15;
        }
        nbytes += (pl->nbytes + 63) & ~(size_t)63;
        nsamples += pl->nsamples;
    }
    if (j->dev_gather) j->ggroups.push_back((uint32_t)j->gsegs.size());
    j->pkt_bytes = pkt_bytes;
    j->nbytes = nbytes;
    j->nsamples = nsamples;
    j->nframes = n;
    return 0;
}

extern "C" int htj2k_job_parse(htj2k_ctx *c, const uint8_t *pkt, int size, htj2k_job **job)
{
    const uint8_t *pk[1] = { pkt };
    int sz[1] = { size };
    if (!pkt) return HTJ2K_ERR_EINVAL;
    return htj2k_job_parse_batch(c, pk, sz, 1, job);
}

extern "C" int htj2k_job_num_frames(const htj2k_job *j) { return j ? j->nframes : HTJ2K_ERR_EINVAL; }

extern "C" int htj2k_job_host_ms(const htj2k_job *j, float *ms_parse, float *ms_stage)
{
    if (!j || j->nframes <= 0) return HTJ2K_ERR_EINVAL;
    float p = 0, s = 0;
    for (int f = 0; f < j->nframes; f++) { p += j->frames[f].ms_parse; s += j->frames[f].ms_stage; }
    if (ms_parse) *ms_parse = p / j->nframes;
    if (ms_stage) *ms_stage = s / j->nframes;
    return 0;
}

extern "C" int htj2k_job_frame_info(const htj2k_job *j, int frame, htj2k_info *info)
{
    if (!j || frame < 0 || frame >= j->nframes || !j->frames[frame].plan || !info) return HTJ2K_ERR_EINVAL;
    *info = j->frames[frame].plan->info;
    return 0;
}
extern "C" int htj2k_job_info(const htj2k_job *j, htj2k_info *info) { return htj2k_job_frame_info(j, 0, info); }
extern "C" int htj2k_job_bytes_consumed(const htj2k_job *j)
{
    return j && j->nframes > 0 && j->frames[0].plan ? j->frames[0].plan->bytes_consumed : HTJ2K_ERR_EINVAL;
}
extern "C" int htj2k_job_num_tilecomps(const htj2k_job *j) { return j && j->nframes ? (int)j->tilecomps.size() : HTJ2K_ERR_EINVAL; }
extern "C" int htj2k_job_num_blocks(const htj2k_job *j) { return j && j->nframes ? (int)j->blocks.size() : HTJ2K_ERR_EINVAL; }
extern "C" int htj2k_job_tilecomp_dims(const htj2k_job *j, int tc, int *w, int *h, int *is_float)
{
    if (!j || !j->nframes || tc < 0 || tc >= (int)j->tilecomps.size()) return HTJ2K_ERR_EINVAL;
    if (w) *w = j->tilecomps[tc].w;
    if (h) *h = j->tilecomps[tc].h;
    if (is_float) *is_float = j->tilecomps[tc].transform == J2K_DWT97;
    return 0;
}

static size_t align_up(size_t v, size_t a) { return (v + a - 1) / a * a; }

static int ht_lds_layout(htj2k_ctx *c, uint32_t max_p, uint32_t max_s, uint32_t max_qw, uint32_t bm_words, HtLds *out, HtLds *out_ext);

static int build_ht_lds(htj2k_ctx *c, const J2kBlock *blocks, int nblocks, const uint8_t *const *bases,
                        const uint32_t *base_of_block, HtLds *out, HtLds *out_ext = nullptr)
{
    uint32_t max_p = 0, max_s = 2, max_qw = 1, bm_words = 0;
    for (int i = 0; i < nblocks; i++) {
        const J2kBlock &b = blocks[i];
        if (!b.npasses) continue;
        uint32_t qw = (b.w + 1u) >> 1;
        if (qw > max_qw) max_qw = qw;
        if (b.lcup >= 2) {
            const uint8_t *D = bases[base_of_block ? base_of_block[i] : 0] + b.data_off;
            uint32_t scup = ((uint32_t)D[b.lcup - 1] << 4) + (D[b.lcup - 2] & 0x0F);
            if (scup >= 2 && scup <= b.lcup && scup <= 4079) {
                if (scup > max_s) max_s = scup;
                if (b.lcup - scup > max_p) max_p = b.lcup - scup;
            }
        }
        int rem = b.npasses % 3, plhd = rem ? b.npasses - rem : b.npasses - 3;
        if (b.npasses - plhd > 1) {
            uint32_t wds = ((uint32_t)(b.w + 2) * (b.h + 2) + 31) / 32 + 1;
            if (wds > bm_words) bm_words = wds;
        }
    }
    return ht_lds_layout(c, max_p, max_s, max_qw, bm_words, out, out_ext);
}

static int ht_lds_layout(htj2k_ctx *c, uint32_t max_p, uint32_t max_s, uint32_t max_qw, uint32_t bm_words, HtLds *out, HtLds *out_ext)
{
    HtLds &L = *out;
    size_t off = 4096;
    L.ms_words = ((max_p * 8 + 31) / 32 + 3 + 3) & ~3u;
    L.off_ms = (uint32_t)off;  off += (size_t)L.ms_words * 4;
    L.vlc_words = (max_s * 8 + 31) / 32 + 2;
    L.off_vlc = (uint32_t)off; off += (size_t)L.vlc_words * 4;
    L.suf_bytes = (uint32_t)align_up(max_s, 4);
    L.off_suf = (uint32_t)off; off += L.suf_bytes;
    L.max_qw = max_qw;
    L.off_qinfo = (uint32_t)off; off += (size_t)2 * max_qw * 4;
    L.off_E = (uint32_t)off;   off += align_up((size_t)2 * (2 * max_qw + 8), 4);
    L.bm_words = bm_words;
    L.off_bm = (uint32_t)off;  off += (size_t)4 * bm_words * 4;
    L.total = (uint32_t)align_up(off, 16);
    if (out_ext) {
        HtLds &X = *out_ext;
        size_t o = 0;
        X = L;
        X.off_ms = 0; o += (size_t)X.ms_words * 4;
        X.off_vlc = (uint32_t)o; X.vlc_words = 0;
        X.off_suf = (uint32_t)o; X.suf_bytes = 0;
        X.off_qinfo = (uint32_t)o; o += (size_t)2 * max_qw * 4;
        X.off_E = (uint32_t)o; o += align_up((size_t)2 * (2 * max_qw + 8), 4);
        X.off_bm = (uint32_t)o; o += (size_t)4 * bm_words * 4;
        X.total = (uint32_t)align_up(o, 16);
    }
    if ((int)L.total > 160 * 1024) {
        clog(c, LOG_ERROR, "a codeblock needs %u bytes of LDS\n", L.total);
        return HTJ2K_ERR_PATCHWELCOME;
    }
    return 0;
}

static size_t ref_layout(const J2kBlock *blocks, size_t nblocks, std::vector<uint32_t> &reflist, std::vector<uint32_t> &roff, uint32_t *max_w,
                         uint32_t *max_h = nullptr)
{
    reflist.clear();
    roff.assign(nblocks + 1, 0);
    *max_w = 0;
    if (max_h) *max_h = 0;
    for (size_t i = 0; i < nblocks; i++) {
        const J2kBlock &b = blocks[i];
        const int rem = b.npasses % 3, plhd = rem ? b.npasses - rem : b.npasses - 3;
        if (b.npasses && !(b.flags & J2K_BLK_PART1) && b.npasses - plhd > 1 && b.w <= 64 && b.roi_shift == 0) {
            reflist.push_back((uint32_t)i);
            if (b.w > *max_w) *max_w = b.w;
            if (max_h && b.h > *max_h) *max_h = b.h;
        }
    }
    size_t nm = 0;
    for (size_t g = 0; g < reflist.size(); g += 64) {
        uint32_t hmax = 0;
        for (size_t l = g; l < std::min(g + 64, reflist.size()); l++) hmax = std::max<uint32_t>(hmax, blocks[reflist[l]].h);
        for (size_t l = g; l < std::min(g + 64, reflist.size()); l++) roff[reflist[l]] = (uint32_t)(nm + (l - g));
        nm += (size_t)HT_REF_STRIDE * 3 * hmax;
    }
    return nm;
}

static void push_bytes(std::vector<uint8_t> &v, const void *p, size_t n)
{
    const uint8_t *b = (const uint8_t *)p;
    v.insert(v.end(), b, b + n);
}

static long pk16_lift_bound(long ll, long hl, long lh, long hh)
{
    const long LIM = 32767;
    bool ok = true;
    auto s1 = [&](long c0, long a) { if (2 * a + 2 > LIM) ok = false; return c0 + (2 * a + 2) / 4; };
    auto s2 = [&](long c0, long a) { if (2 * a > LIM) ok = false; return c0 + a; };
    const long e = s1(ll, hl), o = s2(hl, e);
    const long eh = s1(lh, hh), oh = s2(hh, eh);
    const long re0 = s1(e, eh), ro0 = s2(eh, re0);
    const long re1 = s1(o, oh), ro1 = s2(oh, re1);
    const long m = std::max(std::max(re0, ro0), std::max(re1, ro1));
    return ok && m <= LIM && e <= LIM && o <= LIM && eh <= LIM && oh <= LIM ? m : -1;
}
static bool pk16_bounds(const long (*B)[4], int nc, bool rct)
{
    long bc[3] = { 0, 0, 0 };
    for (int c = 0; c < nc; c++)
        if ((bc[c] = pk16_lift_bound(B[c][0], B[c][1], B[c][2], B[c][3])) < 0) return false;
    if (rct) {
        if (bc[1] + bc[2] > 32767) return false;
        if (bc[0] + (bc[1] + bc[2]) / 4 + 1 > 32767) return false;
    }
    return true;
}

extern "C" long htj2k_pk16_lift_bound(long ll, long hl, long lh, long hh) { return pk16_lift_bound(ll, hl, lh, hh); }
extern "C" int htj2k_pk16_bounds(const long (*b)[4], int nc, int rct) { return b && nc >= 1 && nc <= 3 && pk16_bounds(b, nc, rct != 0) ? 1 : 0; }

static void pk16_eligibility(htj2k_job *j)
{
    j->pk_bits = 0;
    for (LevelLaunch &L : j->launches_fused) L.pk_bits = 0;
    if (!j->coef16_ok) return;
    const int ntc = (int)j->tilecomps.size();
    std::vector<std::pair<uint32_t, int>> start(ntc);
    for (int t = 0; t < ntc; t++) start[t] = { j->tilecomps[t].plane_off, t };
    std::sort(start.begin(), start.end());
    auto plane_of = [&](uint32_t off) {
        auto it = std::upper_bound(start.begin(), start.end(), std::make_pair(off, 1 << 30));
        return it == start.begin() ? -1 : (it - 1)->second;
    };
    std::vector<uint8_t> mb((size_t)ntc * J2K_MAX_DWTLEV * 4, 0);
    for (const J2kBlock &b : j->blocks) {
        const int t = plane_of(b.plane_off);
        if (t < 0) return;
        const J2kTileComp &tc = j->tilecomps[t];
        if (tc.ndeclevels < 1 || tc.ndeclevels > J2K_MAX_DWTLEV || tc.w <= 0) return;
        const uint32_t off = b.plane_off - tc.plane_off;
        const int x = (int)(off % (uint32_t)tc.w), y = (int)(off / (uint32_t)tc.w);
        int lev = tc.ndeclevels - 1, band = 0;
        for (; lev >= 0; lev--) {
            const int mh = tc.mod[lev][0], mv = tc.mod[lev][1];
            const int nlx = ((mh + tc.linelen[lev][0] + 1) >> 1) - ((mh + 1) >> 1), nly = ((mv + tc.linelen[lev][1] + 1) >> 1) - ((mv + 1) >> 1);
            band = (x >= nlx ? 1 : 0) + (y >= nly ? 2 : 0);
            if (band || lev == 0) break;
        }
        uint8_t &m = mb[((size_t)t * J2K_MAX_DWTLEV + lev) * 4 + band];
        if (b.M_b > m) m = b.M_b;
    }
// ... 217 lines not shown
                std::vector<DwtTileArgs> ta;
                for (int t = 0; t < ntc; t++) {
                    const J2kTileComp &tc = j->tilecomps[t];
                    if (!tc.coded || tc.transform != type || lev >= tc.ndeclevels) continue;
                    if (in_group[t] && lev == tc.ndeclevels - 1) continue;
                    const DwtTileArgs a = level_args(tc, lev);
                    ta.push_back(a);
                    g.max_lh = std::max(g.max_lh, a.g.lh); g.max_lv = std::max(g.max_lv, a.g.lv);
                    g.min_l = std::min(g.min_l, std::min(a.g.lh, a.g.lv));
                    g.alg_bytes += 8.0 * a.g.lh * a.g.lv;
                    g.all_fast = g.all_fast && stream_fast_geom(a.g);
                }
                if (!ta.empty()) {
                    g.count = (int)ta.size();
                    while (j->h_desc.size() % 16) j->h_desc.push_back(0);
                    g.table_off = j->h_desc.size();
                    push_bytes(j->h_desc, ta.data(), ta.size() * sizeof(DwtTileArgs));
                    j->launches_fused.push_back(g);
                }
                for (int nc = 1; nc <= 4; nc++)
                for (int outk = -1; outk <= 3; outk++) {
                    LevelLaunch fz = g;
                    fz.count = 0; fz.max_lh = fz.max_lv = 0; fz.alg_bytes = 0; fz.hbm_bytes = 0; fz.min_l = 1 << 30; fz.nc = nc;
                    fz.all_fast = outk >= 0;
                    fz.outk = outk;
                    std::vector<DwtFusedArgs> fa;
                    for (const Group &gr : groups) {
                        const J2kTileComp &tc = j->tilecomps[gr.tc0];
                        if (gr.nc != nc || tc.transform != type || tc.ndeclevels - 1 != lev) continue;
                        {
                            const PackTile *PT0 = (const PackTile *)(j->h_desc.data() + j->pack_off) + gr.pack_tile;
                            const DwtLevel g0 = level_args(tc, lev).g;
                            int kind = stream_fast_geom(g0) ? stream_fast_outk(*PT0, g0, nc, gr.comp0) : -1;
                            if (kind > 0 && type == J2K_DWT97_INT) kind = -1;
                            if (kind != outk) continue;
                        }
                        DwtFusedArgs A;
                        memset(&A, 0, sizeof(A));
                        for (int cc = 0; cc < nc; cc++) A.a[cc] = level_args(j->tilecomps[gr.tc0 + cc], lev);
                        A.ncomp = nc; A.pack_tile = gr.pack_tile; A.comp0 = gr.comp0;
                        fa.push_back(A);
                        fz.max_lh = std::max(fz.max_lh, A.a[0].g.lh); fz.max_lv = std::max(fz.max_lv, A.a[0].g.lv);
                        fz.min_l = std::min(fz.min_l, std::min(A.a[0].g.lh, A.a[0].g.lv));
                        const PackTile *PT = (const PackTile *)(j->h_desc.data() + j->pack_off) + gr.pack_tile;
                        fz.alg_bytes += (double)nc * A.a[0].g.lh * A.a[0].g.lv * 8.0;
                        fz.hbm_bytes += (double)nc * A.a[0].g.lh * A.a[0].g.lv * (4.0 + PT->out_bytes);
                    }
                    if (fa.empty()) continue;
                    fz.count = (int)fa.size();
                    while (j->h_desc.size() % 16) j->h_desc.push_back(0);
                    fz.table_off = j->h_desc.size();
                    push_bytes(j->h_desc, fa.data(), fa.size() * sizeof(DwtFusedArgs));
                    j->launches_fused.push_back(fz);
                }
            }
        for (int t = 0; t < ntc; t++) j->plane_fused[t] = in_group[t];
    }
    j->x3_ok = false;
    {
        const LevelLaunch *L3[3] = { nullptr, nullptr, nullptr };
        for (const LevelLaunch &L : j->launches_fused)
            if (L.type == J2K_DWT53 && L.nc == 0 && L.level < 3) L3[L.level] = &L;
        if (L3[0] && L3[1] && L3[2] && L3[0]->count == L3[1]->count && L3[1]->count == L3[2]->count) {
            bool ok = true;
            double alg = 0, hbm = 0;
            for (int k = 0; k < 3 && ok; k++) {
                const DwtTileArgs *A = (const DwtTileArgs *)(j->h_desc.data() + L3[k]->table_off);
                for (int i = 0; i < L3[k]->count && ok; i++) {
                    ok = stream_fast_geom(A[i].g) && A[i].g.mh == 0 && A[i].g.mv == 0;
                    const double n = (double)A[i].g.lh * A[i].g.lv;
                    alg += 8.0 * n;
                    hbm += 2.0 * n * (k == 0 ? 1.0 : 0.75) + (k == 2 ? 2.0 * n : 0.0);
                }
                j->x3_tab[k] = L3[k]->table_off;
                j->x3_lh[k] = L3[k]->max_lh;
            }
            j->x3_ok = ok;
            j->x3_count = L3[0]->count;
            j->x3_lv2 = L3[2]->max_lv;
            j->x3_alg = alg; j->x3_hbm = hbm;
        }
    }
    (void)c;
    return 0;
}

extern "C" int htj2k_job_upload(htj2k_ctx *c, htj2k_job *j)
{
    if (!c || !j || j->nframes <= 0) return HTJ2K_ERR_EINVAL;
    int r;
    HIP_TRY(c, hipSetDevice(c->device));
    {
        uint32_t max_p = 0, max_s = 2, max_qw = 1, bm_words = 0;
        for (int f = 0; f < j->nframes; f++) {
            const J2kPlan *pl = j->frames[f].plan;
            max_p = std::max(max_p, pl->max_pcup); max_s = std::max(max_s, pl->max_scup);
            max_qw = std::max(max_qw, pl->max_qw); bm_words = std::max(bm_words, pl->max_bm_words);
        }
        if ((r = ht_lds_layout(c, max_p, max_s, max_qw, bm_words, &j->lds, &j->lds_ext)) < 0) return r;
        j->max_qw = j->lds.max_qw;
        j->max_lref = 0;
        for (int f = 0; f < j->nframes; f++) j->max_lref = std::max(j->max_lref, j->frames[f].plan->max_lref);
    }
    {
        auto quads = [](const J2kBlock &b) { return b.npasses ? (uint32_t)((b.w + 1) >> 1) * ((b.h + 1) >> 1) : 0u; };
        const size_t nb = j->blocks.size();
        std::vector<J2kBlock> tmp(nb);
        {
            std::vector<uint32_t> cnt(1026, 0);
            for (const J2kBlock &b : j->blocks) cnt[1024 - std::min<uint32_t>(b.w, 1024) + 1]++;
            for (size_t i = 1; i < cnt.size(); i++) cnt[i] += cnt[i - 1];
            for (const J2kBlock &b : j->blocks) tmp[cnt[1024 - std::min<uint32_t>(b.w, 1024)]++] = b;
        }
        {
            uint32_t maxq = 0;
            for (const J2kBlock &b : tmp) maxq = std::max(maxq, quads(b));
            std::vector<uint32_t> cnt((size_t)maxq + 2, 0);
            for (const J2kBlock &b : tmp) cnt[maxq - quads(b) + 1]++;
            for (size_t i = 1; i < cnt.size(); i++) cnt[i] += cnt[i - 1];
            for (const J2kBlock &b : tmp) j->blocks[cnt[maxq - quads(b)]++] = b;
        }
        {
            auto part1 = [](const J2kBlock &b) { return (b.flags & J2K_BLK_PART1) != 0; };
            auto mid = std::stable_partition(j->blocks.begin(), j->blocks.end(), [&](const J2kBlock &b) { return !part1(b); });
            j->nht = (int)(mid - j->blocks.begin());
            std::stable_sort(mid, j->blocks.end(), [&](const J2kBlock &a, const J2kBlock &b) {
                if ((a.w > 64) != (b.w > 64)) return a.w > 64;
                if (a.h != b.h) return a.h > b.h;
                if (a.w != b.w) return a.w > b.w;
                return a.npasses > b.npasses;
            });
            j->mqwaves.clear();
            j->mq_planes = 1;
            size_t units = 0;
            for (size_t i = (size_t)j->nht; i < j->blocks.size(); i += 64) {
                MqWave W;
                int hmax = 0, wmax = 0, pmax = 0;
                for (size_t k = i; k < std::min(i + 64, j->blocks.size()); k++) {
                    const J2kBlock &b = j->blocks[k];
                    hmax = std::max<int>(hmax, b.h); wmax = std::max<int>(wmax, b.w); pmax = std::max<int>(pmax, b.npasses);
                }
                W.hmax = (uint16_t)hmax; W.wmax = (uint16_t)wmax; W.pmax = (uint16_t)pmax;
                W.rows = (uint16_t)(((hmax + 3) & ~3) + 2);
                W.chunks = (uint16_t)((wmax + 63) / 64);
                W.pad = 0;
                if (units > 0xFFFFFF00ull) return HTJ2K_ERR_PATCHWELCOME;
                W.soff = (uint32_t)units;
                units += (size_t)(4 + std::min((pmax + 1) / 3 + 1, 32)) * W.rows * W.chunks;
                j->mq_planes = std::max<uint32_t>(j->mq_planes, (uint32_t)std::min((pmax + 1) / 3 + 1, 32));
                j->mqwaves.push_back(W);
            }
            j->mq_scratch_units = units;
        }
        j->qoff.resize(j->blocks.size() + 1);
        size_t q = 0;
        for (size_t i = 0; i < j->blocks.size(); i++) {
            j->qoff[i] = (uint32_t)q;
            const J2kBlock &b = j->blocks[i];
            if (b.npasses && !(b.flags & J2K_BLK_PART1)) q += ht_qsym_words(b.w, b.h);
        }
        if (q > 0xFFFFFF00ull) return HTJ2K_ERR_PATCHWELCOME;
        j->nquads = q;
        const size_t nm = ref_layout(j->blocks.data(), j->blocks.size(), j->reflist, j->roff, &j->ref_max_w, &j->ref_max_h);
        if (nm > 0xFFFFFF00ull) return HTJ2K_ERR_PATCHWELCOME;
        j->nrefmasks = nm;
    }
    const size_t coef_bytes = (j->nsamples + 64) * sizeof(uint32_t);
    const int nblocks = (int)j->blocks.size();
    if ((r = j->d_bytes.ensure(j->nbytes + 256)) < 0) return r;
    if (!j->mqwaves.empty() &&
        ((r = j->d_mqwaves.ensure(j->mqwaves.size() * sizeof(MqWave))) < 0 ||
         (r = j->d_mqscratch.ensure(j->mq_scratch_units * 512 + 512)) < 0)) return r;
    if ((r = j->d_blocks.ensure((size_t)(nblocks + 1) * sizeof(J2kBlock))) < 0) return r;
    if ((r = j->d_status.ensure((size_t)(nblocks + 1) * sizeof(int))) < 0) return r;
    if ((r = j->d_coef.ensure(coef_bytes)) < 0) return r;
    if ((r = j->d_t0.ensure(coef_bytes)) < 0) return r;
    if ((r = j->d_t1.ensure(coef_bytes)) < 0) return r;
    if ((r = j->d_qsym.ensure(j->nquads * sizeof(ht_sym_t) + 256 + 8192)) < 0) return r;
    if ((r = j->d_qoff.ensure((j->qoff.size() + 1) * sizeof(uint32_t))) < 0) return r;
    if ((r = j->d_vlcu.ensure(j->nbytes + 16384)) < 0 || (r = j->d_melu.ensure(j->nbytes + 16384)) < 0) return r;
    if ((r = j->d_reflist.ensure((j->reflist.size() + 1) * sizeof(uint32_t))) < 0 ||
        (r = j->d_roff.ensure(j->roff.size() * sizeof(uint32_t))) < 0 ||
        (r = j->d_refbits.ensure((j->nrefmasks + 8) * sizeof(uint64_t))) < 0) return r;
    for (int f = 0; f < j->nframes; f++) {
        FrameSlot &F = j->frames[f];
        const J2kPlan *pl = F.plan;
        memset(&F.out, 0, sizeof(F.out));
        for (int p = 0; p < pl->info.nplanes; p++) {
            const int ls = pl->info.plane_width[p] * pl->info.plane_bytes_per_sample[p];
            if ((r = F.d_out[p].ensure((size_t)ls * pl->info.plane_height[p] + 64)) < 0) return r;
            F.out.ptr[p] = (uint8_t *)F.d_out[p].p;
            F.out.linesize[p] = ls;
            F.out.width[p] = pl->info.plane_width[p];
            F.out.height[p] = pl->info.plane_height[p];
        }
        for (int p = 0; p < pl->info.nplanes && p < 4; p++) {
            if (pl->info.has_palette && p == 1) continue;
            long long covered = 0;
            int first = -1;
            for (int t = 0; t < pl->ntilecomps; t++)
                if (pl->tilecomps[t].out_plane == p && (first < 0 || pl->tilecomps[t].comp < first)) first = pl->tilecomps[t].comp;
            for (int t = 0; t < pl->ntilecomps; t++) {
                const J2kTileComp &tc = pl->tilecomps[t];
                if (tc.out_plane == p && tc.comp == first && tc.out_w > 0 && tc.out_h > 0) covered += (long long)tc.out_w * tc.out_h;
            }
            const long long need = (long long)pl->info.plane_width[p] * pl->info.plane_height[p];
            if (covered < need)
                HIP_TRY(c, hipMemsetAsync(F.d_out[p].p, 0, (size_t)F.out.linesize[p] * F.out.height[p], j->stream));
        }
    }
    if ((r = build_descriptors(c, j)) < 0) return r;
    {
        bool ok = j->nht == (int)j->blocks.size() && j->reflist.empty() && j->tile_ok && j->any_fusable && !j->blocks.empty();
        for (size_t t = 0; ok && t < j->tilecomps.size(); t++) {
            const J2kTileComp &tc = j->tilecomps[t];
            ok = tc.coded && tc.transform == J2K_DWT53 && tc.ndeclevels >= 1;
        }
        for (size_t i = 0; ok && i < j->blocks.size(); i++) {
            const J2kBlock &b = j->blocks[i];
            ok = b.w <= 64 && b.M_b <= 15 && b.roi_shift == 0 && b.i_step == 32768 && (b.flags & 3) == J2K_DWT53;
            if (ok && b.npasses) { const int rem = b.npasses % 3; ok = b.npasses - (rem ? b.npasses - rem : b.npasses - 3) == 1; }
        }
        for (size_t i = 0; ok && i < j->launches_fused.size(); i++) {
            const LevelLaunch &L = j->launches_fused[i];
            ok = L.all_fast && L.type == J2K_DWT53 && L.min_l >= 2;
        }
        for (size_t i = 0; ok && i < j->tile_fusable.size(); i++) ok = j->tile_fusable[i] != 0;
        j->coef16_ok = ok;
        pk16_eligibility(j);
        for (size_t i = 0; ok && i < j->blocks.size(); i++) {
            const J2kBlock &b = j->blocks[i];
            ok = !(b.w & 1) && !(b.stride & 1) && !(b.plane_off & 1);
        }
        j->pair_ok = ok;
        bool mok = j->nht == (int)j->blocks.size() && !j->blocks.empty();
        int maxw = 0;
        const int t0 = mok ? (j->blocks[0].flags & 3) : 0;
        for (size_t i = 0; mok && i < j->blocks.size(); i++) {
            const J2kBlock &b = j->blocks[i];
            mok = b.w <= 64 && b.roi_shift == 0 && (b.flags & 3) == t0;
            if (b.w > maxw) maxw = b.w;
        }
        j->multi_nb = mok ? (maxw <= 32 ? 4 : 2) : 0;
        j->multi_t = t0;
        const size_t multi_lds_max = getenv("HTJ2K_MULTI_LDS") ? (size_t)atoi(getenv("HTJ2K_MULTI_LDS")) : 12 * 1024;
        if (mok && (size_t)j->multi_nb * (j->lds_ext.ms_words + 4) * 4 > multi_lds_max) j->multi_nb = 0;
        if (j->multi_nb && !j->reflist.empty() &&
            (j->ref_max_h > 64 || ht_multi_refine_lds(j->multi_nb, ht_nsp(j->max_lref), j->ref_max_h) > 24 * 1024)) j->multi_nb = 0;
    }
    if ((r = j->d_desc.ensure(j->h_desc.size() + 64)) < 0) return r;
    HIP_TRY(c, hipEventRecord(j->ev[0], j->stream));
    if (j->dev_gather) {
        if ((r = j->d_pkt.ensure(j->pkt_bytes + 256)) < 0 || (r = j->d_lit.ensure(j->lit.size() + 64)) < 0 ||
            (r = j->d_gsegs.ensure((j->gsegs.size() + 1) * sizeof(J2kSeg))) < 0 ||
            (r = j->d_ggroups.ensure((j->ggroups.size() + 1) * sizeof(uint32_t))) < 0) return r;
        if (!j->pkt_h2d_issued)
            for (int f = 0; f < j->nframes; f++)
                HIP_TRY(c, job_packet_h2d(j, j->frames[f], (size_t)j->frames[f].plan->pkt_size));
        j->pkt_h2d_issued = false;
        if (!j->lit.empty())
            HIP_TRY(c, hipMemcpyAsync(j->d_lit.p, j->lit.data(), j->lit.size(), hipMemcpyHostToDevice, j->stream));
        if (!j->gsegs.empty())
            HIP_TRY(c, hipMemcpyAsync(j->d_gsegs.p, j->gsegs.data(), j->gsegs.size() * sizeof(J2kSeg), hipMemcpyHostToDevice, j->stream));
        HIP_TRY(c, hipMemcpyAsync(j->d_ggroups.p, j->ggroups.data(), j->ggroups.size() * sizeof(uint32_t), hipMemcpyHostToDevice, j->stream));
        HIP_TRY(c, hipMemsetAsync(j->d_bytes.p, 0, j->nbytes + 256, j->stream));
        const int ngroups = (int)j->ggroups.size() - 1;
        if (ngroups > 0 && !j->gsegs.empty()) {
            hipLaunchKernelGGL(k_gather, dim3((ngroups + 3) / 4), dim3(256), 0, j->stream, (const J2kSeg *)j->d_gsegs.p,
                               (const uint32_t *)j->d_ggroups.p, ngroups, (const uint8_t *)j->d_pkt.p, (const uint8_t *)j->d_lit.p,
                               (uint8_t *)j->d_bytes.p);
            HIP_TRY(c, hipGetLastError());
        }
    } else {
        for (int f = 0; f < j->nframes; f++) {
            const FrameSlot &F = j->frames[f];
            if (F.plan->nbytes)
                HIP_TRY(c, hipMemcpyAsync((uint8_t *)j->d_bytes.p + F.bytes_base, F.plan->bytes, F.plan->nbytes,
                                          hipMemcpyHostToDevice, j->stream));
        }
    }
    for (int f = 0; f < j->nframes; f++) {
        const FrameSlot &F = j->frames[f];
        if (F.plan->info.has_palette && F.plan->info.nplanes > 1)
            HIP_TRY(c, hipMemcpyAsync(F.out.ptr[1], F.plan->palette, 256 * sizeof(uint32_t), hipMemcpyHostToDevice, j->stream));
    }
    if (nblocks) {
        HIP_TRY(c, hipMemcpyAsync(j->d_blocks.p, j->blocks.data(), (size_t)nblocks * sizeof(J2kBlock), hipMemcpyHostToDevice, j->stream));
        HIP_TRY(c, hipMemcpyAsync(j->d_qoff.p, j->qoff.data(), j->qoff.size() * sizeof(uint32_t), hipMemcpyHostToDevice, j->stream));
        HIP_TRY(c, hipMemcpyAsync(j->d_roff.p, j->roff.data(), j->roff.size() * sizeof(uint32_t), hipMemcpyHostToDevice, j->stream));
        if (!j->reflist.empty())
            HIP_TRY(c, hipMemcpyAsync(j->d_reflist.p, j->reflist.data(), j->reflist.size() * sizeof(uint32_t), hipMemcpyHostToDevice, j->stream));
        if (!j->mqwaves.empty())
            HIP_TRY(c, hipMemcpyAsync(j->d_mqwaves.p, j->mqwaves.data(), j->mqwaves.size() * sizeof(MqWave), hipMemcpyHostToDevice, j->stream));
    }
    HIP_TRY(c, hipEventRecord(j->ev[1], j->stream));
    j->uploaded = 1;
    return 0;
}

static uint32_t *buf_ptr(htj2k_job *j, int which)
{
    return (uint32_t *)(which == 0 ? j->d_coef.p : which == 1 ? j->d_t0.p : j->d_t1.p);
}

template <int TYPE>
static void launch_generic_level(htj2k_job *j, const LevelLaunch &L)
{
    const DwtLevel *tab = (const DwtLevel *)((uint8_t *)j->d_desc.p + L.table_off);
    dim3 gh((L.max_lh + 255) / 256, L.max_lv, L.count), gv((L.max_lh + 255) / 256, L.max_lv, L.count);
    hipLaunchKernelGGL((k_idwt_h<TYPE>), gh, dim3(256), 0, j->stream, tab, (const uint32_t *)j->d_coef.p, (uint32_t *)j->d_t0.p);
    hipLaunchKernelGGL((k_idwt_v<TYPE>), gv, dim3(256), 0, j->stream, tab, (const uint32_t *)j->d_t0.p, (uint32_t *)j->d_coef.p);
}

#define TILE_W 64
#define TILE_H 32

static int stream_strip_rows(int max_lh, int max_lv, int count)
{
    const char *e = getenv("HTJ2K_STRIP");
    if (e && atoi(e) >= 8) return atoi(e) & ~1;
    const long cols = (max_lh + STREAM_TW - 1) / STREAM_TW;
    return cols * ((max_lv + 15) / 16) * count >= 2048 ? 16 : 8;
}

static int stream_strip_cols(int max_lh, int out_bytes)
{
    const char *e = getenv(out_bytes == 2 ? "HTJ2K_TW16" : out_bytes == 4 ? "HTJ2K_TW32" : "HTJ2K_TWF");
    if (e && atoi(e) >= 64 && atoi(e) <= STREAM_TW) return atoi(e) & ~3;
    if (out_bytes == 2) return max_lh >= 1920 ? 224 : STREAM_TW;
    if (out_bytes == 4 || out_bytes == 6) return max_lh >= 960 ? 224 : STREAM_TW;
    return STREAM_TW;
}

static StreamGrid stream_grid(int max_lh, int max_lv, int th, int count, int tw = STREAM_TW, int wpb = 1)
{
    StreamGrid G;
    G.tw = tw;
    G.gx = (max_lh + tw - 1) / tw;
    G.gy = (max_lv + th - 1) / th;
    G.nstrips = G.gx * G.gy * count;
    G.per_xcd = ((G.nstrips + 7) / 8 + wpb - 1) / wpb * wpb;
    return G;
}
static int stream_wpb(int max_lh, int tw)
{
    const int e = getenv("HTJ2K_WPB") ? atoi(getenv("HTJ2K_WPB")) : 0;
    if (e >= 1 && e <= 8) return e;
    return std::max(1, std::min(8, (max_lh + tw - 1) / tw));
}
static int stream_occ_lds(int wpb)
{
    const int e = getenv("HTJ2K_OCC_LDS") ? atoi(getenv("HTJ2K_OCC_LDS")) : 0;
    return std::min(e * wpb, 48 * 1024);
}
static int stream_pk_lds(int wpb)
{
    const int e = getenv("HTJ2K_PK_LDS") ? atoi(getenv("HTJ2K_PK_LDS")) : -1;
    if (e >= 0) return e;
    const int per_cu = wpb >= 8 ? 2 : wpb >= 4 ? 3 : 12 / wpb;
    return (160 * 1024 / per_cu) & ~1023;
}

template <int TYPE>
static void launch_tile_generic(const void *tab, int max_lh, int max_lv, int min_l, int count, int mode, hipStream_t s,
                                const uint32_t *ll, const uint32_t *band, uint32_t *out, bool all_fast, int coef16 = 0)
{
    if (mode >= 3 && min_l >= 2) {
        const int th = stream_strip_rows(max_lh, max_lv, count);
        const int tw = stream_strip_cols(max_lh, all_fast ? 4 : 0);
        const int wpb = all_fast || (TYPE == J2K_DWT53 && coef16) ? stream_wpb(max_lh, tw) : 1;
        const StreamGrid G = stream_grid(max_lh, max_lv, th, count, tw, wpb);
        const dim3 g(8 * G.per_xcd / wpb), blk(64 * wpb);
        const int lds = stream_occ_lds(wpb);
        if (TYPE == J2K_DWT53 && coef16 == 2) hipLaunchKernelGGL((k_idwt_stream<J2K_DWT53, true, true, true>), g, blk, lds, s, (const DwtTileArgs *)tab, ll, band, out, th, G);
        else if (TYPE == J2K_DWT53 && coef16 == 1) hipLaunchKernelGGL((k_idwt_stream<J2K_DWT53, true, true, false>), g, blk, lds, s, (const DwtTileArgs *)tab, ll, band, out, th, G);
        else if (all_fast) hipLaunchKernelGGL((k_idwt_stream<TYPE, true>), g, blk, lds, s, (const DwtTileArgs *)tab, ll, band, out, th, G);
        else hipLaunchKernelGGL((k_idwt_stream<TYPE, false>), g, dim3(64), 0, s, (const DwtTileArgs *)tab, ll, band, out, th, G);
    } else {
        dim3 g((max_lh + TILE_W - 1) / TILE_W, (max_lv + TILE_H - 1) / TILE_H, count);
        hipLaunchKernelGGL((k_idwt_tile<TYPE, TILE_W, TILE_H>), g, dim3(256), 0, s, (const DwtTileArgs *)tab, ll, band, out);
    }
}

static hipError_t launch_unstuff(hipStream_t st, const J2kBlock *blocks, int nblocks, const uint8_t *bytes, uint32_t *vlcu, uint32_t *melu,
                                 uint32_t us_words, int g)
{
    const size_t us_lds = (size_t)us_words * 4;
    hipError_t e = hipSuccess;
    if (g >= 4 && 4 * us_lds <= 64 * 1024) {
        if (4 * us_lds > 48 * 1024) e = hipFuncSetAttribute((const void *)k_ht_unstuff_g<16>, hipFuncAttributeMaxDynamicSharedMemorySize, (int)(4 * us_lds));
        if (e == hipSuccess) hipLaunchKernelGGL(k_ht_unstuff_g<16>, dim3((nblocks + 3) / 4), dim3(64), 4 * us_lds, st, blocks, nblocks, bytes, vlcu, melu, us_words);
    } else if (g >= 2 && 2 * us_lds <= 64 * 1024) {
        if (2 * us_lds > 48 * 1024) e = hipFuncSetAttribute((const void *)k_ht_unstuff_g<32>, hipFuncAttributeMaxDynamicSharedMemorySize, (int)(2 * us_lds));
        if (e == hipSuccess) hipLaunchKernelGGL(k_ht_unstuff_g<32>, dim3((nblocks + 1) / 2), dim3(64), 2 * us_lds, st, blocks, nblocks, bytes, vlcu, melu, us_words);
    } else {
        if (us_lds > 48 * 1024) e = hipFuncSetAttribute((const void *)k_ht_unstuff, hipFuncAttributeMaxDynamicSharedMemorySize, (int)us_lds);
        if (e == hipSuccess) hipLaunchKernelGGL(k_ht_unstuff, dim3(nblocks), dim3(64), us_lds, st, blocks, nblocks, bytes, vlcu, melu, us_words);
    }
    return e;
}

static int ll16_check_bits(const htj2k_ctx *c, const htj2k_job *j)
{
    return std::min(c->ll16_test_bits, c->idwt_pk && j->pk_bits ? j->pk_bits : 16);
}

template <int TYPE>
static void launch_tile_level(htj2k_ctx *c, htj2k_job *j, const LevelLaunch &L, const uint32_t *ll, uint32_t *out)
{
    if (TYPE == J2K_DWT53 && j->ll16_run && c->idwt_mode >= 3 && L.min_l >= 2) {
        const int th = stream_strip_rows(L.max_lh, L.max_lv, L.count);
        const int tw = stream_strip_cols(L.max_lh, 2), wpb = stream_wpb(L.max_lh, tw);
        const StreamGrid G = stream_grid(L.max_lh, L.max_lv, th, L.count, tw, wpb);
        if (L.pk_bits && j->pk_run)
            hipLaunchKernelGGL(k_idwt_stream_ll16<true>, dim3(8 * G.per_xcd / wpb), dim3(64 * wpb), 0, j->stream,
                               (const DwtTileArgs *)((uint8_t *)j->d_desc.p + L.table_off), ll, (const uint32_t *)j->d_coef.p, out, th, G,
                               (int *)j->d_status.p + j->blocks.size(), ll16_check_bits(c, j));
        else
            hipLaunchKernelGGL(k_idwt_stream_ll16<false>, dim3(8 * G.per_xcd / wpb), dim3(64 * wpb), 0, j->stream,
                               (const DwtTileArgs *)((uint8_t *)j->d_desc.p + L.table_off), ll, (const uint32_t *)j->d_coef.p, out, th, G,
                               (int *)j->d_status.p + j->blocks.size(), ll16_check_bits(c, j));
        return;
    }
    launch_tile_generic<TYPE>((uint8_t *)j->d_desc.p + L.table_off, L.max_lh, L.max_lv, L.min_l, L.count, c->idwt_mode,
                              j->stream, ll, (const uint32_t *)j->d_coef.p, out, L.all_fast,
                              j->coef_is16 ? (L.level == 0 ? 2 : 1) : 0);
}

template <int TYPE>
static void launch_fused_level(htj2k_job *j, const LevelLaunch &L, const uint32_t *ll)
{
    const int th = stream_strip_rows(L.max_lh, L.max_lv, L.count);
    const int tw = stream_strip_cols(L.max_lh, L.outk == 0 ? 3 : L.outk == 1 ? 6 : L.outk == 2 ? 1 : L.outk == 3 ? 2 : 0);
    const bool multi = (TYPE == J2K_DWT53 && j->coef_is16) || (TYPE != J2K_DWT97_INT && (L.outk >= 1 || (L.nc == 3 && L.all_fast)));
    const int wpb = multi ? stream_wpb(L.max_lh, tw) : 1;
    const int occ_lds = stream_occ_lds(wpb);
    const StreamGrid G = stream_grid(L.max_lh, L.max_lv, th, L.count, tw, wpb);
    dim3 g(8 * G.per_xcd / wpb);
    const dim3 blk(64 * wpb);
    const DwtFusedArgs *tab = (const DwtFusedArgs *)((uint8_t *)j->d_desc.p + L.table_off);
    const PackTile *tiles = (const PackTile *)((uint8_t *)j->d_desc.p + j->pack_off);
    const uint32_t *band = (const uint32_t *)j->d_coef.p;
#define FUSED_FAST(NC_, C16_, LL16_, K_) hipLaunchKernelGGL((k_idwt_stream_pack<TYPE == J2K_DWT97_INT && (K_) ? J2K_DWT53 : TYPE, NC_, true, C16_, LL16_, K_>), g, blk, occ_lds, j->stream, tab, ll, band, tiles, th, G)
    if (TYPE == J2K_DWT53 && j->coef_is16) {
        const bool l0 = L.level == 0 || j->ll16_run;
        const bool pk = l0 && L.pk_bits && j->pk_run;
        const int pk_lds = pk ? stream_pk_lds(wpb) : 0;
        if (pk && (L.outk == 0 || L.outk == 2)) j->pk_used = L.level == 0 ? 16 : std::min(16, j->pk_bits);
        if (pk && L.outk == 0) {
            if (pk_lds > 48 * 1024)
                (void)hipFuncSetAttribute((const void *)k_idwt_stream_pack<J2K_DWT53, 3, true, true, true, 0, true>, hipFuncAttributeMaxDynamicSharedMemorySize, pk_lds);
            hipLaunchKernelGGL((k_idwt_stream_pack<J2K_DWT53, 3, true, true, true, 0, true>), g, blk, pk_lds, j->stream, tab, ll, band, tiles, th, G);
        } else if (pk && L.outk == 2) {
            if (pk_lds > 48 * 1024)
                (void)hipFuncSetAttribute((const void *)k_idwt_stream_pack<J2K_DWT53, 1, true, true, true, 2, true>, hipFuncAttributeMaxDynamicSharedMemorySize, pk_lds);
            hipLaunchKernelGGL((k_idwt_stream_pack<J2K_DWT53, 1, true, true, true, 2, true>), g, blk, pk_lds, j->stream, tab, ll, band, tiles, th, G);
        }
        else if (L.outk == 0) { if (l0) FUSED_FAST(3, true, true, 0); else FUSED_FAST(3, true, false, 0); }
        else if (L.outk == 1) { if (l0) FUSED_FAST(3, true, true, 1); else FUSED_FAST(3, true, false, 1); }
        else if (L.outk == 2) { if (l0) FUSED_FAST(1, true, true, 2); else FUSED_FAST(1, true, false, 2); }
        else { if (l0) FUSED_FAST(1, true, true, 3); else FUSED_FAST(1, true, false, 3); }
    } else if (L.outk == 1) FUSED_FAST(3, false, false, 1);
    else if (L.outk == 2) FUSED_FAST(1, false, false, 2);
    else if (L.outk == 3) FUSED_FAST(1, false, false, 3);
    else if (L.nc == 1) hipLaunchKernelGGL((k_idwt_stream_pack<TYPE, 1, false>), g, dim3(64), 0, j->stream, tab, ll, band, tiles, th, G);
    else if (L.nc == 3 && L.all_fast) hipLaunchKernelGGL((k_idwt_stream_pack<TYPE, 3, true>), g, blk, occ_lds, j->stream, tab, ll, band, tiles, th, G);
    else if (L.nc == 3) hipLaunchKernelGGL((k_idwt_stream_pack<TYPE, 3, false>), g, dim3(64), 0, j->stream, tab, ll, band, tiles, th, G);
    else hipLaunchKernelGGL((k_idwt_stream_pack<TYPE, 4, false>), g, dim3(64), 0, j->stream, tab, ll, band, tiles, th, G);
}

static hipEvent_t lev_event(htj2k_job *j)
{
    if (j->lev_ev_used >= (int)j->lev_ev.size()) {
        hipEvent_t e = nullptr;
        if (hipEventCreate(&e) != hipSuccess) return nullptr;
        j->lev_ev.push_back(e);
    }
    return j->lev_ev[j->lev_ev_used++];
}

static int run_idwt(htj2k_ctx *c, htj2k_job *j, bool use_tile, bool fuse)
{
    j->lev_ev_used = 0;
    j->lev_bytes.clear();
    j->lev_hbm.clear();
    j->pk_run = c->idwt_pk != 0;
    j->pk_used = 0;
    const std::vector<LevelLaunch> &LL = fuse ? j->launches_fused : use_tile ? j->launches_tile : j->launches_generic;
    bool x3 = false;
    if (fuse && j->ll16_run && j->x3_ok && c->idwt_x3) {
        const int th = getenv("HTJ2K_X3_TH") ? std::max(8, atoi(getenv("HTJ2K_X3_TH")) & ~3) : 24;
        const size_t lds = ((size_t)x3_win0_rows(th) * j->x3_lh[0] + (size_t)x3_win1_rows(th) * j->x3_lh[1]) * sizeof(uint16_t);
        if (lds <= 64 * 1024) {
            x3 = true;
            const int nbands = (j->x3_lv2 + th - 1) / th, total = nbands * j->x3_count;
            hipEvent_t e0 = lev_event(j);
            if (e0) (void)hipEventRecord(e0, j->stream);
            bool x3pk = j->pk_run;
            for (const LevelLaunch &L : LL)
                if (L.type == J2K_DWT53 && L.nc == 0 && L.level < 3 && !L.pk_bits) x3pk = false;
            auto kern = x3pk ? k_idwt_stream_ll16_x3<true> : k_idwt_stream_ll16_x3<false>;
            if (lds > 48 * 1024)
                (void)hipFuncSetAttribute((const void *)kern, hipFuncAttributeMaxDynamicSharedMemorySize, (int)lds);
            hipLaunchKernelGGL(kern, dim3(8 * ((total + 7) / 8)), dim3(256), lds, j->stream,
                               (const DwtTileArgs *)((uint8_t *)j->d_desc.p + j->x3_tab[0]), (const DwtTileArgs *)((uint8_t *)j->d_desc.p + j->x3_tab[1]),
                               (const DwtTileArgs *)((uint8_t *)j->d_desc.p + j->x3_tab[2]), (const uint32_t *)j->d_coef.p, buf_ptr(j, 1),
                               th, nbands, j->x3_count, j->x3_lh[0], j->x3_lh[1], (int *)j->d_status.p + j->blocks.size(), ll16_check_bits(c, j));
            hipEvent_t e1 = lev_event(j);
            if (e1) (void)hipEventRecord(e1, j->stream);
            j->lev_bytes.push_back(j->x3_alg);
            j->lev_hbm.push_back(j->x3_hbm);
        }
    }
    for (const LevelLaunch &L : LL) {
        if (x3 && L.type == J2K_DWT53 && L.nc == 0 && L.level < 3) continue;
        hipEvent_t e0 = lev_event(j);
        if (e0) (void)hipEventRecord(e0, j->stream);
        if (L.nc) {
            const uint32_t *ll = buf_ptr(j, L.level == 0 ? 0 : 1 + ((L.level - 1) & 1));
            if (L.type == J2K_DWT53) launch_fused_level<J2K_DWT53>(j, L, ll);
            else if (L.type == J2K_DWT97) launch_fused_level<J2K_DWT97>(j, L, ll);
            else launch_fused_level<J2K_DWT97_INT>(j, L, ll);
        } else if (!use_tile) {
            if (L.type == J2K_DWT53) launch_generic_level<J2K_DWT53>(j, L);
            else if (L.type == J2K_DWT97) launch_generic_level<J2K_DWT97>(j, L);
            else launch_generic_level<J2K_DWT97_INT>(j, L);
        } else {
            const uint32_t *ll = buf_ptr(j, L.level == 0 ? 0 : 1 + ((L.level - 1) & 1));
            uint32_t *out = buf_ptr(j, 1 + (L.level & 1));
            if (L.type == J2K_DWT53) launch_tile_level<J2K_DWT53>(c, j, L, ll, out);
            else if (L.type == J2K_DWT97) launch_tile_level<J2K_DWT97>(c, j, L, ll, out);
            else launch_tile_level<J2K_DWT97_INT>(c, j, L, ll, out);
        }
        hipEvent_t e1 = lev_event(j);
        if (e1) (void)hipEventRecord(e1, j->stream);
        j->lev_bytes.push_back(L.alg_bytes);
        double hb = L.nc ? L.hbm_bytes : L.alg_bytes;
        if (j->coef_is16) hb -= L.alg_bytes / 8.0 * ((L.level == 0 || j->ll16_run) ? 2.0 : 1.5);
        if (j->ll16_run && !L.nc) hb -= L.alg_bytes / 8.0 * 2.0;
        j->lev_hbm.push_back(hb);
    }
    return 0;
}

extern "C" int htj2k_job_run_stages(htj2k_ctx *c, htj2k_job *j, int mask)
{
    if (!c || !j || j->nframes <= 0 || !j->uploaded) return HTJ2K_ERR_EINVAL;
    const int nall = (int)j->blocks.size(), ntc = (int)j->tilecomps.size();
    const int nblocks = j->nht;
    HIP_TRY(c, hipSetDevice(c->device));
    if (mask & 1) {
        HIP_TRY(c, hipEventRecord(j->ev[2], j->stream));
        if (nall) HIP_TRY(c, hipMemsetAsync(j->d_status.p, 0, ((size_t)nall + 1) * sizeof(int), j->stream));
        if (nall > nblocks) {
            const uint32_t area = mq_lds_area(j->mq_planes);
            unsigned nwide = 0;
            while (nwide < j->mqwaves.size() && j->mqwaves[nwide].chunks > 1) nwide++;
            const unsigned nnarrow = (unsigned)j->mqwaves.size() - nwide;
            if (nwide)
                hipLaunchKernelGGL(k_mq_decode<true>, dim3(nwide), dim3(64), area + MQ_LDS_TABLES, j->stream,
                                   (const J2kBlock *)j->d_blocks.p + nblocks, nall - nblocks, (const uint8_t *)j->d_bytes.p,
                                   (uint32_t *)j->d_coef.p, (int *)j->d_status.p + nblocks, (const MqWave *)j->d_mqwaves.p,
                                   (uint64_t *)j->d_mqscratch.p, area);
            if (nnarrow)
                hipLaunchKernelGGL(k_mq_decode<false>, dim3(nnarrow), dim3(64), area + MQ_LDS_TABLES, j->stream,
                                   (const J2kBlock *)j->d_blocks.p + nblocks + 64 * (size_t)nwide, nall - nblocks - 64 * (int)nwide,
                                   (const uint8_t *)j->d_bytes.p, (uint32_t *)j->d_coef.p, (int *)j->d_status.p + nblocks + 64 * (size_t)nwide,
                                   (const MqWave *)j->d_mqwaves.p + nwide, (uint64_t *)j->d_mqscratch.p, area);
            HIP_TRY(c, hipGetLastError());
        }
        j->coef_is16 = false;
        if (nblocks) {
            const bool vlc_narrow = j->max_qw <= 32;
            const size_t vlc_lds = vlc_narrow ? (size_t)HT_VLC2_LDS : ht_vlc_lds_bytes(j->max_qw);
            j->coef_is16 = c->coef16 && j->coef16_ok && c->ht_mode == 1 && vlc_lds <= 160 * 1024 && mask == 7 &&
                           c->idwt_mode == 3 && c->fuse_pack;
            if (c->ht_mode == 1 && vlc_lds <= 160 * 1024) {
                if (vlc_lds > 48 * 1024)
                    HIP_TRY(c, hipFuncSetAttribute((const void *)k_ht_vlc, hipFuncAttributeMaxDynamicSharedMemorySize, (int)vlc_lds));
                if ((int)j->lds_ext.total > 48 * 1024)
                    HIP_TRY(c, hipFuncSetAttribute((const void *)k_ht_decode<true>, hipFuncAttributeMaxDynamicSharedMemorySize, (int)j->lds_ext.total));
                const uint32_t us_words = 2 * std::max(j->lds.vlc_words, j->reflist.empty() ? 0u : ht_nsp(j->max_lref));
                const int us_g = getenv("HTJ2K_UNSTUFF_G") ? atoi(getenv("HTJ2K_UNSTUFF_G")) : (j->max_qw <= 16 ? 4 : 2);
                HIP_TRY(c, launch_unstuff(j->stream, (const J2kBlock *)j->d_blocks.p, nblocks, (const uint8_t *)j->d_bytes.p,
                                          (uint32_t *)j->d_vlcu.p, (uint32_t *)j->d_melu.p, us_words, us_g));
                const int vlc_wg = vlc_narrow ? 64 * HT_VLC_NARROW_WAVES : 64;
                if (vlc_narrow)
                    hipLaunchKernelGGL(k_ht_vlc2, dim3((nblocks + vlc_wg - 1) / vlc_wg), dim3(vlc_wg), HT_VLC2_LDS, j->stream,
                                       (const J2kBlock *)j->d_blocks.p, nblocks, (const uint8_t *)j->d_bytes.p,
                                       (const uint16_t *)c->d_tables, (ht_sym_t *)j->d_qsym.p, (const uint32_t *)j->d_qoff.p,
                                       (const uint32_t *)j->d_vlcu.p, (uint32_t *)j->d_qsym.p + j->nquads / 2 + 32);
                else
                hipLaunchKernelGGL(k_ht_vlc, dim3((nblocks + vlc_wg - 1) / vlc_wg), dim3(vlc_wg), vlc_lds, j->stream,
                                   (const J2kBlock *)j->d_blocks.p, nblocks, (const uint8_t *)j->d_bytes.p,
                                   (const uint16_t *)c->d_tables, (ht_sym_t *)j->d_qsym.p, (const uint32_t *)j->d_qoff.p, j->max_qw,
                                   (const uint32_t *)j->d_vlcu.p, (const uint32_t *)j->d_melu.p, (uint32_t *)j->d_qsym.p + j->nquads / 2 + 32);
                const bool multi_run = !(j->coef_is16 && j->pair_ok && c->ht_pair) && !j->coef_is16 && j->multi_nb && c->ht_multi;
                if (!j->reflist.empty()) {
                    auto kref = j->ref_max_w <= 32 ? (multi_run ? k_ht_refine<uint32_t, false> : k_ht_refine<uint32_t, true>)
                                                   : (multi_run ? k_ht_refine<uint64_t, false> : k_ht_refine<uint64_t, true>);
                    hipLaunchKernelGGL(kref, dim3(((unsigned)j->reflist.size() + 63) / 64), dim3(64), 0, j->stream,
                                       (const J2kBlock *)j->d_blocks.p, (const uint32_t *)j->d_reflist.p, (int)j->reflist.size(),
                                       (const uint8_t *)j->d_bytes.p, (const ht_sym_t *)j->d_qsym.p, (const uint32_t *)j->d_qoff.p,
                                       (const uint32_t *)j->d_vlcu.p, (const uint32_t *)j->d_melu.p,
                                       (uint64_t *)j->d_refbits.p, (const uint32_t *)j->d_roff.p);
                }
                j->ht_bpw = (j->coef_is16 && j->pair_ok && c->ht_pair) ? 2 : (!j->coef_is16 && j->multi_nb && c->ht_multi) ? j->multi_nb : 1;
                if (j->coef_is16 && j->pair_ok && c->ht_pair)
                    hipLaunchKernelGGL(k_ht_decode_pair, dim3((nblocks + 1) / 2), dim3(64), 2 * (j->lds_ext.ms_words + 4) * 4, j->stream,
                                       (const J2kBlock *)j->d_blocks.p, nblocks, (const uint8_t *)j->d_bytes.p,
                                       (uint32_t *)j->d_coef.p, (int *)j->d_status.p, j->lds_ext.ms_words,
                                       (const ht_sym_t *)j->d_qsym.p, (const uint32_t *)j->d_qoff.p,
                                       (uint32_t *)j->d_coef.p + j->nsamples + 32);
                else if (!j->coef_is16 && j->multi_nb && c->ht_multi) {
                    const int nb = j->multi_nb;
                    const uint32_t mr_words = j->reflist.empty() ? 0u : ht_nsp(j->max_lref), rg_rows = j->reflist.empty() ? 0u : j->ref_max_h;
                    const size_t lds = (size_t)nb * (j->lds_ext.ms_words + 4) * 4 + (j->reflist.empty() ? 0 : ht_multi_refine_lds(nb, mr_words, rg_rows));
#define HT_MULTI_R(NB_, T_, R_) do { \
                        if (lds > 48 * 1024) HIP_TRY(c, hipFuncSetAttribute((const void *)k_ht_decode_multi<NB_, T_, R_>, hipFuncAttributeMaxDynamicSharedMemorySize, (int)lds)); \
                        hipLaunchKernelGGL((k_ht_decode_multi<NB_, T_, R_>), dim3((nblocks + NB_ - 1) / NB_), dim3(64), lds, j->stream, \
                                           (const J2kBlock *)j->d_blocks.p, nblocks, (const uint8_t *)j->d_bytes.p, \
                                           (uint32_t *)j->d_coef.p, (int *)j->d_status.p, j->lds_ext.ms_words, \
                                           (const ht_sym_t *)j->d_qsym.p, (const uint32_t *)j->d_qoff.p, \
                                           (uint32_t *)j->d_coef.p + j->nsamples + 32, \
                                           (const uint64_t *)j->d_refbits.p, (const uint32_t *)j->d_roff.p, \
                                           (const uint32_t *)j->d_melu.p, mr_words, rg_rows); } while (0)
#define HT_MULTI(NB_, T_) do { if (j->reflist.empty()) HT_MULTI_R(NB_, T_, false); else HT_MULTI_R(NB_, T_, true); } while (0)
                    if (nb == 4) {
                        if (j->multi_t == J2K_DWT53) HT_MULTI(4, J2K_DWT53); else if (j->multi_t == J2K_DWT97) HT_MULTI(4, J2K_DWT97); else HT_MULTI(4, J2K_DWT97_INT);
                    } else {
                        if (j->multi_t == J2K_DWT53) HT_MULTI(2, J2K_DWT53); else if (j->multi_t == J2K_DWT97) HT_MULTI(2, J2K_DWT97); else HT_MULTI(2, J2K_DWT97_INT);
                    }
#undef HT_MULTI
#undef HT_MULTI_R
                } else
                hipLaunchKernelGGL(k_ht_decode<true>, dim3(nblocks), dim3(64), j->lds_ext.total, j->stream,
                                   (const J2kBlock *)j->d_blocks.p, nblocks, (const uint8_t *)j->d_bytes.p,
                                   (uint32_t *)j->d_coef.p, (const uint16_t *)c->d_tables, (int *)j->d_status.p, j->lds_ext,
                                   (const ht_sym_t *)j->d_qsym.p, (const uint32_t *)j->d_qoff.p,
                                   (uint32_t *)j->d_coef.p + j->nsamples + 32,
                                   (const uint64_t *)j->d_refbits.p, (const uint32_t *)j->d_roff.p, j->coef_is16 ? 1 : 0);
            } else {
                j->ht_bpw = 1;
                if ((int)j->lds.total > 48 * 1024)
                    HIP_TRY(c, hipFuncSetAttribute((const void *)k_ht_decode<false>, hipFuncAttributeMaxDynamicSharedMemorySize, (int)j->lds.total));
                hipLaunchKernelGGL(k_ht_decode<false>, dim3(nblocks), dim3(64), j->lds.total, j->stream,
                                   (const J2kBlock *)j->d_blocks.p, nblocks, (const uint8_t *)j->d_bytes.p,
                                   (uint32_t *)j->d_coef.p, (const uint16_t *)c->d_tables, (int *)j->d_status.p, j->lds,
                                   (const ht_sym_t *)nullptr, (const uint32_t *)nullptr, (uint32_t *)j->d_coef.p + j->nsamples + 32,
                                   (const uint64_t *)nullptr, (const uint32_t *)nullptr);
            }
            HIP_TRY(c, hipGetLastError());
        }
        HIP_TRY(c, hipEventRecord(j->ev[3], j->stream));
    }
    if (mask & 6) {
        const bool use_tile = c->idwt_mode != 0 && j->tile_ok;
        const bool fuse = use_tile && c->idwt_mode == 3 && c->fuse_pack && (mask & 6) == 6 && j->any_fusable;
        if (mask & 2)
            for (int t = 0; t < ntc; t++) j->final_eff[t] = use_tile ? j->final_buf[t] : 0;
        j->fused_last = fuse;
        PackTile *T = (PackTile *)(j->h_desc.data() + j->pack_off);
        int ti = 0;
        for (int f = 0; f < j->nframes; f++) {
            const FrameSlot &F = j->frames[f];
            for (int k = 0; k < F.plan->ntiles; k++, ti++) {
                T[ti].fused = fuse && j->tile_fusable[ti];
                for (int cc = 0; cc < T[ti].ncomp; cc++) {
                    const int t = F.tc_base + k * T[ti].ncomp + cc;
                    T[ti].c[cc].src = buf_ptr(j, j->final_eff[t]) + j->tilecomps[t].plane_off;
                }
            }
        }
        if (!(mask & 1)) HIP_TRY(c, hipEventRecord(j->ev[3], j->stream));
        if (j->h_desc != j->h_desc_dev) {
            HIP_TRY(c, hipMemcpyAsync(j->d_desc.p, j->h_desc.data(), j->h_desc.size(), hipMemcpyHostToDevice, j->stream));
            j->h_desc_dev = j->h_desc;
        }
        if (mask & 2) {
            j->ll16_run = c->ll16 && j->coef_is16 && fuse && use_tile && !j->force_ll32;
            j->ll16_checked = !j->ll16_run;
            int r = run_idwt(c, j, use_tile, fuse);
            if (r < 0) return r;
            HIP_TRY(c, hipGetLastError());
        }
        HIP_TRY(c, hipEventRecord(j->ev[4], j->stream));
    }
    if (mask & 4) {
        bool all_fused = j->fused_last;
        for (size_t i = 0; all_fused && i < j->tile_fusable.size(); i++) all_fused = j->tile_fusable[i] != 0;
        if (j->npack && j->pack_maxw > 0 && j->pack_maxh > 0 && !all_fused) {
            dim3 g((j->pack_maxw + 1023) / 1024, j->pack_maxh, j->npack);
            hipLaunchKernelGGL(k_mct_pack, g, dim3(256), 0, j->stream,
                               (const PackTile *)((uint8_t *)j->d_desc.p + j->pack_off));
            HIP_TRY(c, hipGetLastError());
        }
        HIP_TRY(c, hipEventRecord(j->ev[5], j->stream));
    }
    j->ran |= mask;
    return 0;
}

extern "C" int htj2k_job_run(htj2k_ctx *c, htj2k_job *j) { return htj2k_job_run_stages(c, j, 7); }

static int job_settle(htj2k_ctx *c, htj2k_job *j)
{
    HIP_TRY(c, hipStreamSynchronize(j->stream));
    if (j->ll16_checked) return 0;
    j->ll16_checked = true;
    int flag = 0;
    HIP_TRY(c, hipMemcpy(&flag, (const int *)j->d_status.p + j->blocks.size(), sizeof(int), hipMemcpyDeviceToHost));
    if (!flag) return 0;
    clog(c, LOG_INFO, "an LL band left the 16-bit range: inverse DWT run again with 32-bit LL bands\n");
    j->ll16_fallbacks++;
    j->force_ll32 = true;
    const int r = htj2k_job_run_stages(c, j, 6);
    j->force_ll32 = false;
    if (r < 0) return r;
    HIP_TRY(c, hipStreamSynchronize(j->stream));
    return 0;
}

extern "C" int htj2k_job_wait(htj2k_ctx *c, htj2k_job *j)
{
    if (!c || !j) return HTJ2K_ERR_EINVAL;
    return job_settle(c, j);
}

extern "C" int htj2k_job_idwt_packed(const htj2k_job *j) { return j ? j->pk_used : HTJ2K_ERR_EINVAL; }
extern "C" int htj2k_job_ll16(const htj2k_job *j) { return j ? (j->ll16_run ? 1 : (j->ll16_fallbacks ? 2 : 0)) : HTJ2K_ERR_EINVAL; }

extern "C" int htj2k_job_stage_ms(htj2k_ctx *c, htj2k_job *j, float *ms_ht, float *ms_idwt, float *ms_pack)
{
    if (!c || !j) return HTJ2K_ERR_EINVAL;
    HIP_TRY(c, hipStreamSynchronize(j->stream));
    float a = 0, b = 0, d = 0;
    if (j->ran & 1) (void)hipEventElapsedTime(&a, j->ev[2], j->ev[3]);
    if (j->ran & 2) (void)hipEventElapsedTime(&b, j->ev[3], j->ev[4]);
    if (j->ran & 4) (void)hipEventElapsedTime(&d, j->ev[4], j->ev[5]);
    if (ms_ht) *ms_ht = a;
    if (ms_idwt) *ms_idwt = b;
    if (ms_pack) *ms_pack = d;
    return 0;
}
// ... 340 lines not shown
            hipLaunchKernelGGL(k_copy_linear, dim3(grids[g]), dim3(256), 0, s, (const uint4 *)src.p, (uint4 *)dst.p, n);
        (void)hipEventRecord(e1, s);
        e = hipStreamSynchronize(s);
        float ms = 0;
        if (e == hipSuccess) e = hipEventElapsedTime(&ms, e0, e1);
        if (e == hipSuccess && ms > 0) best = std::max(best, (float)(2.0 * n * 16 * iters / (ms * 1e-3) / 1e9));
    }
    if (e == hipSuccess) e = hipGetLastError();
    if (e0) (void)hipEventDestroy(e0);
    if (e1) (void)hipEventDestroy(e1);
    if (s) (void)hipStreamDestroy(s);
    src.release(); dst.release();
    if (e != hipSuccess) { clog(c, LOG_ERROR, "HIP error %s in htj2k_copy_bench\n", hipGetErrorString(e)); return HTJ2K_ERR_EXTERNAL; }
    *gbps = best;
    return 0;
}

extern "C" int htj2k_mct_planes(htj2k_ctx *c, void *p0, void *p1, void *p2, int csize, int type)
{
    if (!c || !p0 || !p1 || !p2 || csize <= 0 || type < 0 || type > 2) return HTJ2K_ERR_EINVAL;
    HIP_TRY(c, hipSetDevice(c->device));
    DevBuf d[3];
    void *h[3] = { p0, p1, p2 };
    int r = 0;
    hipError_t e = hipSuccess;
    for (int i = 0; i < 3 && r >= 0; i++) r = d[i].ensure((size_t)csize * 4);
    for (int i = 0; i < 3 && r >= 0 && e == hipSuccess; i++) e = hipMemcpy(d[i].p, h[i], (size_t)csize * 4, hipMemcpyHostToDevice);
    if (r >= 0 && e == hipSuccess) {
        hipLaunchKernelGGL(k_mct_only, dim3((csize + 255) / 256), dim3(256), 0, 0, (uint32_t *)d[0].p, (uint32_t *)d[1].p, (uint32_t *)d[2].p, csize, type);
        e = hipDeviceSynchronize();
    }
    for (int i = 0; i < 3 && r >= 0 && e == hipSuccess; i++) e = hipMemcpy(h[i], d[i].p, (size_t)csize * 4, hipMemcpyDeviceToHost);
    for (int i = 0; i < 3; i++) d[i].release();
    if (r < 0) return r;
    return e == hipSuccess ? 0 : HTJ2K_ERR_EXTERNAL;
}

static bool block_desc_ok(const J2kBlock &b, size_t nsamples)
{
    if (!b.w || !b.h || b.w > 1024 || b.h > 1024 || (uint32_t)b.w * b.h > 4096 || b.stride < b.w) return false;
    if ((size_t)b.plane_off + (size_t)(b.h - 1) * b.stride + b.w > nsamples) return false;
    if (b.roi_shift > 30 || b.npasses >= 100) return false;
    return true;
}

extern "C" int htj2k_mq_blocks(htj2k_ctx *c, const void *blocks_in, int nblocks, const uint8_t *bytes_in, size_t nbytes_in,
                               void *coef, size_t nsamples, int *status)
{
    if (!c || !blocks_in || nblocks <= 0 || !bytes_in || !coef) return HTJ2K_ERR_EINVAL;
    HIP_TRY(c, hipSetDevice(c->device));
    std::vector<J2kBlock> blk((const J2kBlock *)blocks_in, (const J2kBlock *)blocks_in + nblocks);
    std::vector<uint8_t> pool(16, 0);
    for (int i = 0; i < nblocks; i++) {
        J2kBlock &b = blk[i];
        if (!(b.flags & J2K_BLK_PART1) || !block_desc_ok(b, nsamples) || b.M_b > 37) return HTJ2K_ERR_EINVAL;
        const size_t len = J2K_P1_TRAILER_OFF(b.lcup) + 4 + 2 * (size_t)b.lref;
        if ((size_t)b.data_off + len > nbytes_in) return HTJ2K_ERR_EINVAL;
        {
            const J2kPart1Trailer *tr = (const J2kPart1Trailer *)(bytes_in + b.data_off + J2K_P1_TRAILER_OFF(b.lcup));
            if (tr->nterm != b.lref || tr->bandpos > 3) return HTJ2K_ERR_EINVAL;
            for (uint32_t k = 0; k < tr->nterm; k++)
                if (tr->start[k] > b.lcup) return HTJ2K_ERR_EINVAL;
        }
        const size_t o = pool.size();
        pool.resize(o + J2K_P1_REGION(b.lcup, b.lref), 0);
        memcpy(pool.data() + o, bytes_in + b.data_off, len);
        b.data_off = (uint32_t)o;
    }
    pool.resize(pool.size() + 256, 0);
    std::vector<MqWave> waves;
    size_t units = 0;
    uint32_t planes = 1;
    bool wide = false;
    for (int i = 0; i < nblocks; i += 64) {
        MqWave W;
        int hmax = 0, wmax = 0, pmax = 0;
        for (int k = i; k < std::min(i + 64, nblocks); k++) {
            hmax = std::max<int>(hmax, blk[k].h); wmax = std::max<int>(wmax, blk[k].w); pmax = std::max<int>(pmax, blk[k].npasses);
        }
        const int np = std::min((pmax + 1) / 3 + 1, 32);
        W.hmax = (uint16_t)hmax; W.wmax = (uint16_t)wmax; W.pmax = (uint16_t)pmax;
        W.rows = (uint16_t)(((hmax + 3) & ~3) + 2);
        W.chunks = (uint16_t)((wmax + 63) / 64); W.pad = 0;
        W.soff = (uint32_t)units;
        units += (size_t)(4 + np) * W.rows * W.chunks;
        planes = std::max<uint32_t>(planes, (uint32_t)np);
        wide = wide || W.chunks > 1;
        waves.push_back(W);
    }
    DevBuf db, dby, dc, ds, dw, dsc;
    auto release_all = [&]() { db.release(); dby.release(); dc.release(); ds.release(); dw.release(); dsc.release(); };
    int r;
    if ((r = db.ensure((size_t)nblocks * sizeof(J2kBlock))) < 0 || (r = dby.ensure(pool.size())) < 0 ||
        (r = dc.ensure(nsamples * 4 + 64)) < 0 || (r = ds.ensure((size_t)nblocks * 4)) < 0 ||
        (r = dw.ensure(waves.size() * sizeof(MqWave))) < 0 || (r = dsc.ensure(units * 512 + 512)) < 0) {
        release_all();
        return r;
    }
    hipError_t e = hipMemcpy(db.p, blk.data(), (size_t)nblocks * sizeof(J2kBlock), hipMemcpyHostToDevice);
    if (e == hipSuccess) e = hipMemcpy(dby.p, pool.data(), pool.size(), hipMemcpyHostToDevice);
    if (e == hipSuccess) e = hipMemcpy(dc.p, coef, nsamples * 4, hipMemcpyHostToDevice);
    if (e == hipSuccess) e = hipMemset(ds.p, 0, (size_t)nblocks * 4);
    if (e == hipSuccess) e = hipMemcpy(dw.p, waves.data(), waves.size() * sizeof(MqWave), hipMemcpyHostToDevice);
    if (e == hipSuccess) {
        const uint32_t area = mq_lds_area(planes);
        auto kern = wide ? k_mq_decode<true> : k_mq_decode<false>;
        hipLaunchKernelGGL(kern, dim3((unsigned)waves.size()), dim3(64), area + MQ_LDS_TABLES, 0, (const J2kBlock *)db.p, nblocks,
                           (const uint8_t *)dby.p, (uint32_t *)dc.p, (int *)ds.p, (const MqWave *)dw.p, (uint64_t *)dsc.p, area);
        e = hipDeviceSynchronize();
    }
    if (e == hipSuccess) e = hipGetLastError();
    if (e == hipSuccess) e = hipMemcpy(coef, dc.p, nsamples * 4, hipMemcpyDeviceToHost);
    if (e == hipSuccess && status) e = hipMemcpy(status, ds.p, (size_t)nblocks * 4, hipMemcpyDeviceToHost);
    release_all();
    if (e != hipSuccess) { clog(c, LOG_ERROR, "HIP error %s in htj2k_mq_blocks\n", hipGetErrorString(e)); return HTJ2K_ERR_EXTERNAL; }
    return 0;
}

extern "C" int htj2k_ht_blocks(htj2k_ctx *c, const void *blocks_in, int nblocks, const uint8_t *bytes_in, size_t nbytes_in,
                               void *coef, size_t nsamples, int *status)
{
    if (!c || !blocks_in || nblocks <= 0 || !bytes_in || !coef) return HTJ2K_ERR_EINVAL;
    HIP_TRY(c, hipSetDevice(c->device));
    std::vector<J2kBlock> blk((const J2kBlock *)blocks_in, (const J2kBlock *)blocks_in + nblocks);
    std::vector<uint8_t> pool(16, 0);
    for (int i = 0; i < nblocks; i++) {
        J2kBlock &b = blk[i];
        const size_t len = (size_t)b.lcup + b.lref;
        if ((b.flags & J2K_BLK_PART1) || !block_desc_ok(b, nsamples) || b.M_b > 30) return HTJ2K_ERR_EINVAL;
        if ((size_t)b.data_off + len > nbytes_in) return HTJ2K_ERR_EINVAL;
        const size_t o = pool.size();
        pool.resize(o + J2K_BLOCK_REGION(len), 0);
        memcpy(pool.data() + o, bytes_in + b.data_off, len);
        b.data_off = (uint32_t)o;
    }
    const void *blocks = blk.data();
    const uint8_t *bytes = pool.data();
    const size_t nbytes = pool.size();
    struct { HtLds lds, ext; } tmp;
    const uint8_t *bases[1] = { bytes };
    int r = build_ht_lds(c, (const J2kBlock *)blocks, nblocks, bases, nullptr, &tmp.lds, &tmp.ext);
    if (r < 0) return r;
    std::vector<uint32_t> qoff(nblocks + 1);
    size_t nq = 0;
    for (int i = 0; i < nblocks; i++) {
        const J2kBlock &b = ((const J2kBlock *)blocks)[i];
        qoff[i] = (uint32_t)nq;
        if (b.npasses) nq += ht_qsym_words(b.w, b.h);
    }
    std::vector<uint32_t> reflist, roff;
    uint32_t max_lref = 0, ref_max_w = 0;
    for (int i = 0; i < nblocks; i++) max_lref = std::max<uint32_t>(max_lref, ((const J2kBlock *)blocks)[i].lref);
    const size_t nmasks = ref_layout((const J2kBlock *)blocks, (size_t)nblocks, reflist, roff, &ref_max_w);
    DevBuf db, dby, dc, ds, dq, dqo, du[2], drl, dro, drb;
    auto release_all = [&]() {
        db.release(); dby.release(); dc.release(); ds.release(); dq.release(); dqo.release(); du[0].release(); du[1].release();
        drl.release(); dro.release(); drb.release();
    };
    if ((r = dq.ensure((nq + 64) * 4)) < 0 || (r = dqo.ensure((size_t)(nblocks + 1) * 4)) < 0 ||
        (r = du[0].ensure(nbytes + 16384)) < 0 || (r = du[1].ensure(nbytes + 16384)) < 0 ||
        (r = db.ensure((size_t)nblocks * sizeof(J2kBlock))) < 0 || (r = dby.ensure(nbytes + 64)) < 0 ||
        (r = dc.ensure(nsamples * 4 + 64)) < 0 || (r = ds.ensure((size_t)nblocks * 4)) < 0 ||
        (r = drl.ensure((reflist.size() + 1) * 4)) < 0 || (r = dro.ensure(roff.size() * 4)) < 0 ||
        (r = drb.ensure((nmasks + 8) * 8)) < 0) {
        release_all();
        return r;
    }
    hipError_t e = hipMemcpy(db.p, blocks, (size_t)nblocks * sizeof(J2kBlock), hipMemcpyHostToDevice);
    if (e == hipSuccess) e = hipMemcpy(dby.p, bytes, nbytes, hipMemcpyHostToDevice);
    if (e == hipSuccess) e = hipMemcpy(dc.p, coef, nsamples * 4, hipMemcpyHostToDevice);
    if (e == hipSuccess) e = hipMemset(ds.p, 0, (size_t)nblocks * 4);
    if (e == hipSuccess) e = hipMemcpy(dqo.p, qoff.data(), (size_t)nblocks * 4, hipMemcpyHostToDevice);
    if (e == hipSuccess) e = hipMemcpy(dro.p, roff.data(), roff.size() * 4, hipMemcpyHostToDevice);
    if (e == hipSuccess && !reflist.empty()) e = hipMemcpy(drl.p, reflist.data(), reflist.size() * 4, hipMemcpyHostToDevice);
    const size_t vlc_lds = ht_vlc_lds_bytes(tmp.lds.max_qw);
    if (e == hipSuccess && c->ht_mode == 1 && vlc_lds <= 160 * 1024) {
        if (vlc_lds > 48 * 1024)
            e = hipFuncSetAttribute((const void *)k_ht_vlc, hipFuncAttributeMaxDynamicSharedMemorySize, (int)vlc_lds);
        if (e == hipSuccess && (int)tmp.ext.total > 48 * 1024)
            e = hipFuncSetAttribute((const void *)k_ht_decode<true>, hipFuncAttributeMaxDynamicSharedMemorySize, (int)tmp.ext.total);
        if (e == hipSuccess) {
            const uint32_t us_words = 2 * std::max(tmp.lds.vlc_words, reflist.empty() ? 0u : ht_nsp(max_lref));
            e = launch_unstuff(0, (const J2kBlock *)db.p, nblocks, (const uint8_t *)dby.p, (uint32_t *)du[0].p, (uint32_t *)du[1].p, us_words,
                               getenv("HTJ2K_UNSTUFF_G") ? atoi(getenv("HTJ2K_UNSTUFF_G")) : 1);
            hipLaunchKernelGGL(k_ht_vlc, dim3((nblocks + 63) / 64), dim3(64), vlc_lds, 0, (const J2kBlock *)db.p, nblocks,
                               (const uint8_t *)dby.p, (const uint16_t *)c->d_tables, (ht_sym_t *)dq.p, (const uint32_t *)dqo.p,
                               tmp.lds.max_qw, (const uint32_t *)du[0].p, (const uint32_t *)du[1].p, (uint32_t *)dq.p + nq / 2 + 32);
            if (!reflist.empty())
                hipLaunchKernelGGL((ref_max_w <= 32 ? k_ht_refine<uint32_t, true> : k_ht_refine<uint64_t, true>), dim3(((unsigned)reflist.size() + 63) / 64), dim3(64), 0, 0,
                                   (const J2kBlock *)db.p, (const uint32_t *)drl.p, (int)reflist.size(), (const uint8_t *)dby.p,
                                   (const ht_sym_t *)dq.p, (const uint32_t *)dqo.p, (const uint32_t *)du[0].p, (const uint32_t *)du[1].p,
                                   (uint64_t *)drb.p, (const uint32_t *)dro.p);
            hipLaunchKernelGGL(k_ht_decode<true>, dim3(nblocks), dim3(64), tmp.ext.total, 0, (const J2kBlock *)db.p, nblocks,
                               (const uint8_t *)dby.p, (uint32_t *)dc.p, (const uint16_t *)c->d_tables, (int *)ds.p, tmp.ext,
                               (const ht_sym_t *)dq.p, (const uint32_t *)dqo.p, (uint32_t *)dc.p + nsamples + 8,
                               (const uint64_t *)drb.p, (const uint32_t *)dro.p);
            e = hipDeviceSynchronize();
        }
    } else if (e == hipSuccess) {
        if ((int)tmp.lds.total > 48 * 1024)
            e = hipFuncSetAttribute((const void *)k_ht_decode<false>, hipFuncAttributeMaxDynamicSharedMemorySize, (int)tmp.lds.total);
        if (e == hipSuccess) {
            hipLaunchKernelGGL(k_ht_decode<false>, dim3(nblocks), dim3(64), tmp.lds.total, 0, (const J2kBlock *)db.p, nblocks,
                               (const uint8_t *)dby.p, (uint32_t *)dc.p, (const uint16_t *)c->d_tables, (int *)ds.p, tmp.lds,
                               (const ht_sym_t *)nullptr, (const uint32_t *)nullptr, (uint32_t *)dc.p + nsamples + 8,
                               (const uint64_t *)nullptr, (const uint32_t *)nullptr);
            e = hipDeviceSynchronize();
        }
    }
    if (e == hipSuccess) e = hipGetLastError();
    if (e == hipSuccess) e = hipMemcpy(coef, dc.p, nsamples * 4, hipMemcpyDeviceToHost);
    if (e == hipSuccess && status) e = hipMemcpy(status, ds.p, (size_t)nblocks * 4, hipMemcpyDeviceToHost);
    release_all();
    if (e != hipSuccess) { clog(c, LOG_ERROR, "HIP error %s in htj2k_ht_blocks\n", hipGetErrorString(e)); return HTJ2K_ERR_EXTERNAL; }
    return 0;
}
```

Before: 169,300 Mpixel/s.

## Interleave unstuffed VLC words across 64-block groups for coalesced narrow VLC reads

Adds an interleaved layout for the unstuffed VLC stream: each group of 64 codeblocks shares rows of 512 words, with 8 consecutive words per block per row. In the narrow VLC kernel each lane handles one block, so its 16-byte loads now land next to its neighbours' and coalesce. The unstuff kernels write into this layout and remap their workgroup order so that blocks sharing a row are processed together. The cost is an extra host-side layout pass, a new device buffer sized by the largest Lcup in each group, and bounds clipping in the VLC reader.

```diff
diff --git a/ffmpeg-ht_amd/csrc/ht_kernels.hpp b/ffmpeg-ht_amd/csrc/ht_kernels.hpp
--- a/ffmpeg-ht_amd/csrc/ht_kernels.hpp
+++ b/ffmpeg-ht_amd/csrc/ht_kernels.hpp
@@ -26,6 +26,20 @@
 typedef uint16_t ht_sym_t;
 __host__ __device__ inline uint32_t ht_nsw(uint32_t Scup) { return (Scup * 8 + 31) / 32 + 2; }
 __host__ __device__ inline uint32_t ht_nsp(uint32_t Lref) { return (Lref * 8 + 31) / 32 + 3; }
+
+#define HT_IL_ROW_WORDS 512
+__host__ __device__ inline size_t ht_il_word(uint32_t row0, int L, uint32_t w)
+{
+    return ((size_t)row0 + (w >> 3)) * HT_IL_ROW_WORDS + (uint32_t)L * 8u + (w & 7u);
+}
+__host__ __device__ inline uint32_t ht_il_rows(uint32_t lcup) { return (ht_nsw(lcup < 4079u ? lcup : 4079u) + 7u) >> 3; }
+template <int R>
+__device__ __forceinline__ uint32_t ht_il_wg(uint32_t b, uint32_t n)
+{
+    if (R == 1 || b >= n - n % (8u * R)) return b;
+    const uint32_t r = b % (8u * R);
+    return b - r + (r & 7u) * R + (r >> 3);
+}
 
 __host__ __device__ inline uint32_t ht_sym_pack_fields(uint32_t rho, uint32_t ek, uint32_t e1)
 {
@@ -1564,12 +1578,13 @@
 template <int LPB>
 __global__ void __launch_bounds__(64)
 k_ht_unstuff_g(const J2kBlock *__restrict__ blocks, int nblocks, const uint8_t *__restrict__ bytes,
-               uint32_t *__restrict__ vlc_u, uint32_t *__restrict__ mel_u, uint32_t lds_words)
+               uint32_t *__restrict__ vlc_u, uint32_t *__restrict__ mel_u, uint32_t lds_words,
+               const uint32_t *__restrict__ il_row0, uint32_t *__restrict__ vlc_il)
 {
     extern __shared__ __align__(16) uint32_t sw[];
     constexpr int G = 64 / LPB;
     const int lane = threadIdx.x, gl = lane & (LPB - 1);
-    const int bi = (int)blockIdx.x * G + lane / LPB;
+    const int bi = (int)(il_row0 ? ht_il_wg<(G < 4 ? 4 / G : 1)>(blockIdx.x, gridDim.x) : blockIdx.x) * G + lane / LPB;
     J2kBlock b;
     memset(&b, 0, sizeof(b));
     if (bi < nblocks) b = blocks[bi];
@@ -1608,7 +1623,11 @@
         }
     }
     __syncthreads();
-    if (ok) for (uint32_t i = gl; i < nsw; i += LPB) vlO[i] = sv[i];
+    if (ok) {
+        uint32_t *o = il_row0 ? vlc_il + ht_il_word(il_row0[bi >> 6], bi & 63, 0) : vlO;
+        const uint32_t pitch = il_row0 ? HT_IL_ROW_WORDS : 8u;
+        for (uint32_t i = gl; i < nsw; i += LPB) o[(i >> 3) * pitch + (i & 7)] = sv[i];
+    }
 
     const int rem = b.npasses % 3, plhd = rem ? b.npasses - rem : b.npasses - 3;
     const uint32_t Lref = b.lref, nsp = ht_nsp(Lref);
@@ -1645,12 +1664,14 @@
 
 __global__ void __launch_bounds__(64)
 k_ht_unstuff(const J2kBlock *__restrict__ blocks, int nblocks, const uint8_t *__restrict__ bytes,
-             uint32_t *__restrict__ vlc_u, uint32_t *__restrict__ mel_u, uint32_t lds_words)
+             uint32_t *__restrict__ vlc_u, uint32_t *__restrict__ mel_u, uint32_t lds_words,
+             const uint32_t *__restrict__ il_row0, uint32_t *__restrict__ vlc_il)
 {
     extern __shared__ __align__(16) uint32_t sw[];
     const int lane = threadIdx.x;
-    if ((int)blockIdx.x >= nblocks) return;
-    const J2kBlock b = blocks[blockIdx.x];
+    const int bi = (int)(il_row0 ? ht_il_wg<4>(blockIdx.x, gridDim.x) : blockIdx.x);
+    if (bi >= nblocks) return;
+    const J2kBlock b = blocks[bi];
     if (b.npasses == 0 || b.lcup < 2) return;
     const uint8_t *D = bytes + b.data_off;
     const uint32_t Lcup = b.lcup;
@@ -1687,7 +1708,11 @@
     }
 
     __syncthreads();
-    for (uint32_t i = lane; i < nsw; i += 64) vlO[i] = sv[i];
+    {
+        uint32_t *o = il_row0 ? vlc_il + ht_il_word(il_row0[bi >> 6], bi & 63, 0) : vlO;
+        const uint32_t pitch = il_row0 ? HT_IL_ROW_WORDS : 8u;
+        for (uint32_t i = lane; i < nsw; i += 64) o[(i >> 3) * pitch + (i & 7)] = sv[i];
+    }
 
     const int rem = b.npasses % 3, plhd = rem ? b.npasses - rem : b.npasses - 3;
     if (b.npasses - plhd > 1 && b.lref > 0) {
@@ -2169,11 +2194,12 @@
     return ht_uvlc_entry2_from(p1, p2, lp, d1, d2);
 }
 
+template <bool IL>
 __global__ void __launch_bounds__(64 * HT_VLC_NARROW_WAVES)
 k_ht_vlc2(const J2kBlock *__restrict__ blocks, int nblocks, const uint8_t *__restrict__ bytes,
           const uint16_t *__restrict__ g_tables, ht_sym_t *__restrict__ qsym,
           const uint32_t *__restrict__ qoff,
-          const uint32_t *__restrict__ vlc_u, uint32_t *__restrict__ sink)
+          const uint32_t *__restrict__ vlc_u, uint32_t *__restrict__ sink, const uint32_t *__restrict__ il_row0)
 {
     extern __shared__ __align__(16) uint8_t smem[];
     uint16_t *tbl = (uint16_t *)smem;
@@ -2200,6 +2226,7 @@
     ht_sym_t *qout = qsym;
     const uint8_t *mraw = bytes + 16;
     int mlim = 0;
+    uint32_t vlim = 0;
     if (bi < nblocks) {
         const J2kBlock b = blocks[bi];
         bool ok = b.npasses != 0 && b.lcup >= 2;
@@ -2216,6 +2243,7 @@
             doff = b.data_off >> 2;
             mraw = bytes + b.data_off + (b.lcup - Scup);
             mlim = (int)Scup;
+            vlim = ht_nsw(Scup);
         }
     }
     const int ppr = (qw + 1) >> 1;
@@ -2226,7 +2254,11 @@
     const uint32_t my_lo = (uint32_t)(uintptr_t)qout, my_hi = (uint32_t)((uintptr_t)qout >> 32);
     __syncthreads();
 
-    const uint32_t *vsrc = vlc_u + doff;
+    const uint32_t *vsrc = IL ? vlc_u + ht_il_word(qh > 0 ? il_row0[bi >> 6] : 0u, lane, 0) : vlc_u + doff;
+    auto vword = [&](uint32_t w) { return IL ? vsrc + (size_t)(w >> 3) * HT_IL_ROW_WORDS + (w & 7u) : vsrc + w; };
+    auto vclip = [&](uint4 &q, uint32_t w) {
+        q.x = w < vlim ? q.x : 0u; q.y = w + 1 < vlim ? q.y : 0u; q.z = w + 2 < vlim ? q.z : 0u; q.w = w + 3 < vlim ? q.w : 0u;
+    };
     uint32_t vpos = 4;
     uint32_t *vst = vstage + lane * VPITCH;
     uint32_t *ost = ostage + lane * OPITCH;
@@ -2241,8 +2273,9 @@
     if (qh > 0) {
 #pragma unroll
         for (int jx = 0; jx < 4; jx++) {
-            uint4 q;
-            __builtin_memcpy(&q, vsrc + 4 * jx, 16);
+            uint4 q = make_uint4(0u, 0u, 0u, 0u);
+            if ((uint32_t)(4 * jx) < vlim) __builtin_memcpy(&q, vword(4 * jx), 16);
+            vclip(q, 4 * jx);
             vst[4 * jx] = q.x; vst[4 * jx + 1] = q.y; vst[4 * jx + 2] = q.z; vst[4 * jx + 3] = q.w;
             if (jx == 0) { vst[16] = q.x; vst[17] = q.y; }
         }
@@ -2276,6 +2309,7 @@
         const bool pair = MAIN || qx + 1 < qw;
         if ((t & 1) == 0) {
             if (pend) {
+                if (pw + 8 > vlim) { vclip(nxv, pw); vclip(nxw, pw + 4); }
                 uint32_t *r = vst + (pw & 15);
                 r[0] = nxv.x; r[1] = nxv.y; r[2] = nxv.z; r[3] = nxv.w;
                 if (!(pw & 15)) { vst[16] = nxv.x; vst[17] = nxv.y; }
@@ -2284,8 +2318,10 @@
             }
             pend = (int)(hw - (vpos >> 5)) < 8;
             if (pend) {
-                __builtin_memcpy(&nxv, vsrc + hw, 16);
-                __builtin_memcpy(&nxw, vsrc + hw + 4, 16);
+                if (hw < vlim) {
+                    __builtin_memcpy(&nxv, vword(hw), 16);
+                    __builtin_memcpy(&nxw, vword(hw + 4), 16);
+                }
                 pw = hw;
                 hw += 8;
             }
diff --git a/ffmpeg-ht_amd/csrc/htj2k_device.hip b/ffmpeg-ht_amd/csrc/htj2k_device.hip
--- a/ffmpeg-ht_amd/csrc/htj2k_device.hip
+++ b/ffmpeg-ht_amd/csrc/htj2k_device.hip
@@ -102,6 +102,7 @@
     htj2k_job *own_job = nullptr;
     int idwt_mode = 3;
     int fuse_pack = 1;
+    int vlc_il = 1;
     int idwt_x3 = 1;
     int ht_pair = 1;
     int ht_multi = 1;
@@ -182,6 +183,9 @@
     size_t pkt_bytes = 0;
     bool pkt_h2d_issued = false;
     std::vector<uint32_t> qoff;
+    std::vector<uint32_t> il_row0;
+    size_t il_rows = 0;
+    DevBuf d_vlci, d_ilrow0;
     std::vector<uint32_t> reflist, roff;
     size_t nrefmasks = 0;
     uint32_t ref_max_w = 0;
@@ -293,6 +297,8 @@
     if (m && !strcmp(m, "generic")) c->idwt_mode = 0;
     if (m && !strcmp(m, "tile")) c->idwt_mode = 1;
     if (m && !strcmp(m, "stream")) c->idwt_mode = 3;
+    const char *vil = getenv("HTJ2K_VLC_IL");
+    if (vil) c->vlc_il = atoi(vil) ? 1 : 0;
     const char *l16 = getenv("HTJ2K_LL16");
     if (l16) c->ll16 = atoi(l16) ? 1 : 0;
     const char *pk = getenv("HTJ2K_PK");
@@ -323,6 +329,7 @@
     if (!strcmp(name, "coef16")) { c->coef16 = value ? 1 : 0; return 0; }
     if (!strcmp(name, "ht_pair")) { c->ht_pair = value ? 1 : 0; return 0; }
     if (!strcmp(name, "idwt_x3")) { c->idwt_x3 = value ? 1 : 0; return 0; }
+    if (!strcmp(name, "vlc_il")) { c->vlc_il = value ? 1 : 0; return 0; }
     if (!strcmp(name, "idwt_pk")) { c->idwt_pk = value ? 1 : 0; return 0; }
     if (!strcmp(name, "ht_multi")) { c->ht_multi = value ? 1 : 0; return 0; }
     if (!strcmp(name, "ll16")) { c->ll16 = value ? 1 : 0; return 0; }
@@ -363,7 +370,7 @@
     if (j->stream) (void)hipStreamSynchronize(j->stream);
     j->d_bytes.release(); j->d_blocks.release(); j->d_status.release(); j->d_coef.release();
     j->d_t0.release(); j->d_t1.release(); j->d_desc.release(); j->d_qsym.release(); j->d_qoff.release();
-    j->d_vlcu.release(); j->d_melu.release(); j->d_reflist.release(); j->d_roff.release(); j->d_refbits.release();
+    j->d_vlcu.release(); j->d_melu.release(); j->d_vlci.release(); j->d_ilrow0.release(); j->d_reflist.release(); j->d_roff.release(); j->d_refbits.release();
     j->d_mqwaves.release(); j->d_mqscratch.release();
     j->d_pkt.release(); j->d_lit.release(); j->d_gsegs.release(); j->d_ggroups.release();
     for (FrameSlot &f : j->frames) {
@@ -673,6 +680,7 @@
 static size_t align_up(size_t v, size_t a) { return (v + a - 1) / a * a; }
 
 static int ht_lds_layout(htj2k_ctx *c, uint32_t max_p, uint32_t max_s, uint32_t max_qw, uint32_t bm_words, HtLds *out, HtLds *out_ext);
+static size_t il_layout(const J2kBlock *blocks, size_t nblocks, std::vector<uint32_t> &row0);
 
 static int build_ht_lds(htj2k_ctx *c, const J2kBlock *blocks, int nblocks, const uint8_t *const *bases,
                         const uint32_t *base_of_block, HtLds *out, HtLds *out_ext = nullptr)
@@ -1196,6 +1204,9 @@
             }
             j->mq_scratch_units = units;
         }
+        j->il_row0.clear();
+        j->il_rows = il_layout(j->max_qw <= 32 ? j->blocks.data() : nullptr, (size_t)j->nht, j->il_row0);
+        if (j->il_rows > 0xFFFFFF00ull) return HTJ2K_ERR_PATCHWELCOME;
         j->qoff.resize(j->blocks.size() + 1);
         size_t q = 0;
         for (size_t i = 0; i < j->blocks.size(); i++) {
@@ -1223,6 +1234,9 @@
     if ((r = j->d_qsym.ensure(j->nquads * sizeof(ht_sym_t) + 256 + 8192)) < 0) return r;
     if ((r = j->d_qoff.ensure((j->qoff.size() + 1) * sizeof(uint32_t))) < 0) return r;
     if ((r = j->d_vlcu.ensure(j->nbytes + 16384)) < 0 || (r = j->d_melu.ensure(j->nbytes + 16384)) < 0) return r;
+    if (!j->il_row0.empty() &&
+        ((r = j->d_vlci.ensure(j->il_rows * HT_IL_ROW_WORDS * sizeof(uint32_t))) < 0 ||
+         (r = j->d_ilrow0.ensure(j->il_row0.size() * sizeof(uint32_t))) < 0)) return r;
     if ((r = j->d_reflist.ensure((j->reflist.size() + 1) * sizeof(uint32_t))) < 0 ||
         (r = j->d_roff.ensure(j->roff.size() * sizeof(uint32_t))) < 0 ||
         (r = j->d_refbits.ensure((j->nrefmasks + 8) * sizeof(uint64_t))) < 0) return r;
@@ -1332,6 +1346,8 @@
         HIP_TRY(c, hipMemcpyAsync(j->d_blocks.p, j->blocks.data(), (size_t)nblocks * sizeof(J2kBlock), hipMemcpyHostToDevice, j->stream));
         HIP_TRY(c, hipMemcpyAsync(j->d_qoff.p, j->qoff.data(), j->qoff.size() * sizeof(uint32_t), hipMemcpyHostToDevice, j->stream));
         HIP_TRY(c, hipMemcpyAsync(j->d_roff.p, j->roff.data(), j->roff.size() * sizeof(uint32_t), hipMemcpyHostToDevice, j->stream));
+        if (!j->il_row0.empty())
+            HIP_TRY(c, hipMemcpyAsync(j->d_ilrow0.p, j->il_row0.data(), j->il_row0.size() * sizeof(uint32_t), hipMemcpyHostToDevice, j->stream));
         if (!j->reflist.empty())
             HIP_TRY(c, hipMemcpyAsync(j->d_reflist.p, j->reflist.data(), j->reflist.size() * sizeof(uint32_t), hipMemcpyHostToDevice, j->stream));
         if (!j->mqwaves.empty())
@@ -1426,20 +1442,36 @@
     }
 }
 
+static size_t il_layout(const J2kBlock *blocks, size_t nblocks, std::vector<uint32_t> &row0)
+{
+    row0.clear();
+    if (!blocks || !nblocks) return 0;
+    row0.reserve((nblocks + 63) / 64);
+    size_t rows = 0;
+    for (size_t i = 0; i < nblocks; i += 64) {
+        uint32_t lmax = 0;
+        for (size_t k = i; k < std::min(i + 64, nblocks); k++)
+            if (blocks[k].npasses) lmax = std::max<uint32_t>(lmax, blocks[k].lcup);
+        row0.push_back((uint32_t)std::min<size_t>(rows, 0xFFFFFFFFu));
+        rows += ht_il_rows(lmax);
+    }
+    return rows;
+}
+
 static hipError_t launch_unstuff(hipStream_t st, const J2kBlock *blocks, int nblocks, const uint8_t *bytes, uint32_t *vlcu, uint32_t *melu,
-                                 uint32_t us_words, int g)
+                                 uint32_t us_words, int g, const uint32_t *il_row0 = nullptr, uint32_t *vlci = nullptr)
 {
     const size_t us_lds = (size_t)us_words * 4;
     hipError_t e = hipSuccess;
     if (g >= 4 && 4 * us_lds <= 64 * 1024) {
         if (4 * us_lds > 48 * 1024) e = hipFuncSetAttribute((const void *)k_ht_unstuff_g<16>, hipFuncAttributeMaxDynamicSharedMemorySize, (int)(4 * us_lds));
-        if (e == hipSuccess) hipLaunchKernelGGL(k_ht_unstuff_g<16>, dim3((nblocks + 3) / 4), dim3(64), 4 * us_lds, st, blocks, nblocks, bytes, vlcu, melu, us_words);
+        if (e == hipSuccess) hipLaunchKernelGGL(k_ht_unstuff_g<16>, dim3((nblocks + 3) / 4), dim3(64), 4 * us_lds, st, blocks, nblocks, bytes, vlcu, melu, us_words, il_row0, vlci);
     } else if (g >= 2 && 2 * us_lds <= 64 * 1024) {
         if (2 * us_lds > 48 * 1024) e = hipFuncSetAttribute((const void *)k_ht_unstuff_g<32>, hipFuncAttributeMaxDynamicSharedMemorySize, (int)(2 * us_lds));
-        if (e == hipSuccess) hipLaunchKernelGGL(k_ht_unstuff_g<32>, dim3((nblocks + 1) / 2), dim3(64), 2 * us_lds, st, blocks, nblocks, bytes, vlcu, melu, us_words);
+        if (e == hipSuccess) hipLaunchKernelGGL(k_ht_unstuff_g<32>, dim3((nblocks + 1) / 2), dim3(64), 2 * us_lds, st, blocks, nblocks, bytes, vlcu, melu, us_words, il_row0, vlci);
     } else {
         if (us_lds > 48 * 1024) e = hipFuncSetAttribute((const void *)k_ht_unstuff, hipFuncAttributeMaxDynamicSharedMemorySize, (int)us_lds);
-        if (e == hipSuccess) hipLaunchKernelGGL(k_ht_unstuff, dim3(nblocks), dim3(64), us_lds, st, blocks, nblocks, bytes, vlcu, melu, us_words);
+        if (e == hipSuccess) hipLaunchKernelGGL(k_ht_unstuff, dim3(nblocks), dim3(64), us_lds, st, blocks, nblocks, bytes, vlcu, melu, us_words, il_row0, vlci);
     }
     return e;
 }
@@ -1617,6 +1649,7 @@
         if (nblocks) {
             const bool vlc_narrow = j->max_qw <= 32;
             const size_t vlc_lds = vlc_narrow ? (size_t)HT_VLC2_LDS : ht_vlc_lds_bytes(j->max_qw);
+            const bool vlc_il = vlc_narrow && c->vlc_il && !j->il_row0.empty();
             j->coef_is16 = c->coef16 && j->coef16_ok && c->ht_mode == 1 && vlc_lds <= 160 * 1024 && mask == 7 &&
                            c->idwt_mode == 3 && c->fuse_pack;
             if (c->ht_mode == 1 && vlc_lds <= 160 * 1024) {
@@ -1627,13 +1660,15 @@
                 const uint32_t us_words = 2 * std::max(j->lds.vlc_words, j->reflist.empty() ? 0u : ht_nsp(j->max_lref));
                 const int us_g = getenv("HTJ2K_UNSTUFF_G") ? atoi(getenv("HTJ2K_UNSTUFF_G")) : (j->max_qw <= 16 ? 4 : 2);
                 HIP_TRY(c, launch_unstuff(j->stream, (const J2kBlock *)j->d_blocks.p, nblocks, (const uint8_t *)j->d_bytes.p,
-                                          (uint32_t *)j->d_vlcu.p, (uint32_t *)j->d_melu.p, us_words, us_g));
+                                          (uint32_t *)j->d_vlcu.p, (uint32_t *)j->d_melu.p, us_words, us_g,
+                                          vlc_il ? (const uint32_t *)j->d_ilrow0.p : nullptr, (uint32_t *)j->d_vlci.p));
                 const int vlc_wg = vlc_narrow ? 64 * HT_VLC_NARROW_WAVES : 64;
                 if (vlc_narrow)
-                    hipLaunchKernelGGL(k_ht_vlc2, dim3((nblocks + vlc_wg - 1) / vlc_wg), dim3(vlc_wg), HT_VLC2_LDS, j->stream,
+                    hipLaunchKernelGGL((vlc_il ? k_ht_vlc2<true> : k_ht_vlc2<false>), dim3((nblocks + vlc_wg - 1) / vlc_wg), dim3(vlc_wg), HT_VLC2_LDS, j->stream,
                                        (const J2kBlock *)j->d_blocks.p, nblocks, (const uint8_t *)j->d_bytes.p,
                                        (const uint16_t *)c->d_tables, (ht_sym_t *)j->d_qsym.p, (const uint32_t *)j->d_qoff.p,
-                                       (const uint32_t *)j->d_vlcu.p, (uint32_t *)j->d_qsym.p + j->nquads / 2 + 32);
+                                       (const uint32_t *)(vlc_il ? j->d_vlci.p : j->d_vlcu.p), (uint32_t *)j->d_qsym.p + j->nquads / 2 + 32,
+                                       (const uint32_t *)j->d_ilrow0.p);
                 else
                 hipLaunchKernelGGL(k_ht_vlc, dim3((nblocks + vlc_wg - 1) / vlc_wg), dim3(vlc_wg), vlc_lds, j->stream,
                                    (const J2kBlock *)j->d_blocks.p, nblocks, (const uint8_t *)j->d_bytes.p,
@@ -2280,13 +2315,19 @@
     uint32_t max_lref = 0, ref_max_w = 0;
     for (int i = 0; i < nblocks; i++) max_lref = std::max<uint32_t>(max_lref, ((const J2kBlock *)blocks)[i].lref);
     const size_t nmasks = ref_layout((const J2kBlock *)blocks, (size_t)nblocks, reflist, roff, &ref_max_w);
-    DevBuf db, dby, dc, ds, dq, dqo, du[2], drl, dro, drb;
+    std::vector<uint32_t> il_row0;
+    const size_t il_rows = (tmp.lds.max_qw <= 32 && c->vlc_il) ? il_layout((const J2kBlock *)blocks, (size_t)nblocks, il_row0) : 0;
+    if (il_rows > 0xFFFFFF00ull) return HTJ2K_ERR_PATCHWELCOME;
+    const bool vlc_il = !il_row0.empty();
+    DevBuf db, dby, dc, ds, dq, dqo, du[2], dil, dir, drl, dro, drb;
     auto release_all = [&]() {
         db.release(); dby.release(); dc.release(); ds.release(); dq.release(); dqo.release(); du[0].release(); du[1].release();
+        dil.release(); dir.release();
         drl.release(); dro.release(); drb.release();
     };
     if ((r = dq.ensure((nq + 64) * 4)) < 0 || (r = dqo.ensure((size_t)(nblocks + 1) * 4)) < 0 ||
         (r = du[0].ensure(nbytes + 16384)) < 0 || (r = du[1].ensure(nbytes + 16384)) < 0 ||
+        (vlc_il && ((r = dil.ensure(il_rows * HT_IL_ROW_WORDS * 4)) < 0 || (r = dir.ensure(il_row0.size() * 4)) < 0)) ||
         (r = db.ensure((size_t)nblocks * sizeof(J2kBlock))) < 0 || (r = dby.ensure(nbytes + 64)) < 0 ||
         (r = dc.ensure(nsamples * 4 + 64)) < 0 || (r = ds.ensure((size_t)nblocks * 4)) < 0 ||
         (r = drl.ensure((reflist.size() + 1) * 4)) < 0 || (r = dro.ensure(roff.size() * 4)) < 0 ||
@@ -2301,7 +2342,8 @@
     if (e == hipSuccess) e = hipMemcpy(dqo.p, qoff.data(), (size_t)nblocks * 4, hipMemcpyHostToDevice);
     if (e == hipSuccess) e = hipMemcpy(dro.p, roff.data(), roff.size() * 4, hipMemcpyHostToDevice);
     if (e == hipSuccess && !reflist.empty()) e = hipMemcpy(drl.p, reflist.data(), reflist.size() * 4, hipMemcpyHostToDevice);
-    const size_t vlc_lds = ht_vlc_lds_bytes(tmp.lds.max_qw);
+    if (e == hipSuccess && vlc_il) e = hipMemcpy(dir.p, il_row0.data(), il_row0.size() * 4, hipMemcpyHostToDevice);
+    const size_t vlc_lds = vlc_il ? (size_t)HT_VLC2_LDS : ht_vlc_lds_bytes(tmp.lds.max_qw);
     if (e == hipSuccess && c->ht_mode == 1 && vlc_lds <= 160 * 1024) {
         if (vlc_lds > 48 * 1024)
             e = hipFuncSetAttribute((const void *)k_ht_vlc, hipFuncAttributeMaxDynamicSharedMemorySize, (int)vlc_lds);
@@ -2310,7 +2352,14 @@
         if (e == hipSuccess) {
             const uint32_t us_words = 2 * std::max(tmp.lds.vlc_words, reflist.empty() ? 0u : ht_nsp(max_lref));
             e = launch_unstuff(0, (const J2kBlock *)db.p, nblocks, (const uint8_t *)dby.p, (uint32_t *)du[0].p, (uint32_t *)du[1].p, us_words,
-                               getenv("HTJ2K_UNSTUFF_G") ? atoi(getenv("HTJ2K_UNSTUFF_G")) : 1);
+                               getenv("HTJ2K_UNSTUFF_G") ? atoi(getenv("HTJ2K_UNSTUFF_G")) : 1,
+                               vlc_il ? (const uint32_t *)dir.p : nullptr, (uint32_t *)dil.p);
+            if (vlc_il) {
+                const int wg = 64 * HT_VLC_NARROW_WAVES;
+                hipLaunchKernelGGL(k_ht_vlc2<true>, dim3((nblocks + wg - 1) / wg), dim3(wg), HT_VLC2_LDS, 0, (const J2kBlock *)db.p, nblocks,
+                                   (const uint8_t *)dby.p, (const uint16_t *)c->d_tables, (ht_sym_t *)dq.p, (const uint32_t *)dqo.p,
+                                   (const uint32_t *)dil.p, (uint32_t *)dq.p + nq / 2 + 32, (const uint32_t *)dir.p);
+            } else
             hipLaunchKernelGGL(k_ht_vlc, dim3((nblocks + 63) / 64), dim3(64), vlc_lds, 0, (const J2kBlock *)db.p, nblocks,
                                (const uint8_t *)dby.p, (const uint16_t *)c->d_tables, (ht_sym_t *)dq.p, (const uint32_t *)dqo.p,
                                tmp.lds.max_qw, (const uint32_t *)du[0].p, (const uint32_t *)du[1].p, (uint32_t *)dq.p + nq / 2 + 32);
```

Measured after the change: 170,000 Mpixel/s, median of 5. No clear change (+0.4%).
